# orybkin/video-gcp

Measured on AMD Instinct MI355X. Metric: predicted frames/sec, 64x64x3 seq_len=80 gcp_tree (posterior forward + all loss terms, model(inputs) and model.loss() of train.py:157-159, batch-stat BatchNorm), higher is better.
Workload: dtype f32 (encoder / decoder convs and the tree GEMMs from 512 rows: split-f16 MFMA with f32 accumulate, f32-equivalent; everything else exact f32 MFMA)

## Files before the change

### include/gcpx.h

```cpp
#ifndef GCPX_H
#define GCPX_H

#include <stdint.h>

#ifdef __cplusplus
extern "C" {
#endif

#define GCPX_VERSION 1

typedef enum gcpx_status {
    GCPX_OK = 0,
    GCPX_ERR_INVALID_ARG = -1,
    GCPX_ERR_UNSUPPORTED = -2,
    GCPX_ERR_HIP = -3,
    GCPX_ERR_COMM = -4
} gcpx_status;

typedef enum gcpx_act { GCPX_ACT_NONE = 0, GCPX_ACT_LRELU = 1, GCPX_ACT_TANH = 2 } gcpx_act;

int gcpx_version(void);
const char* gcpx_last_error(void);
int gcpx_conv_grid(void);

typedef struct gcpx_conv_src {
    const float* ptr;
    const float* scale;
    const float* shift;
    int32_t C;
    int32_t frame_div;
    int32_t act;
    int32_t _pad;
} gcpx_conv_src;

typedef enum gcpx_head_mode {
    GCPX_HEAD_RAW = 0,
    GCPX_HEAD_DLM_MEAN = 1,
    GCPX_HEAD_DLM_BOTH = 2,
    GCPX_HEAD_TANH_NCHW = 3,
    GCPX_HEAD_DLM_NLL = 4,
    GCPX_HEAD_DLM_NLL_GRAD = 5
} gcpx_head_mode;

typedef struct gcpx_conv_args {
    gcpx_conv_src src[2];
    int32_t nsrc;
    int32_t F;
    int32_t Hin, Win;
    int32_t Hout, Wout;
    int32_t Cin;
    int32_t Cout;
    int32_t out_pitch;
    int32_t upsample;
    int32_t out_act;
    int32_t head_mode;
    const float* wpk;
    const float* bias;
    float* out;
    float* images;
    float* stats_partial;
    const int32_t* raw_row_map;
    const int32_t* src_row_map;
    const int32_t* src_row_frames;
    int32_t n_src_rows;
    int32_t w_split_log2;
    const void* wpk_split;
    const int32_t* w_split_log2_dev;
    int32_t split_layout;
    int32_t nll_rows;
    const float* nll_target;
    float* nll_partial;
    const float* nll_row_weight;
    float nll_scale;
    int32_t _pad3;
    float* images_rows;
    int64_t images_rows_dup;
    const float* bwd_r;
    const float *bwd_scale, *bwd_shift, *bwd_mean, *bwd_rstd;
    const float* addend;
    int32_t addend_frame_div;
    int32_t _pad4;
} gcpx_conv_args;

typedef enum gcpx_split_layout { GCPX_SPLIT_PLAIN = 0, GCPX_SPLIT_ROWFOLD = 1, GCPX_SPLIT_HEAD32 = 2 } gcpx_split_layout;

int gcpx_conv3x3(const gcpx_conv_args* a, void* stream);
int gcpx_conv3x3_grid(const gcpx_conv_args* a);
int gcpx_conv4x4s2(const gcpx_conv_args* a, void* stream);
int gcpx_conv4x4s2_grid(void);
int gcpx_conv4x4s2_image(const float* x, const float* wpk, const float* bias, float* out,
                         int32_t F, int32_t Hin, int32_t Win, int32_t Cout, int32_t out_act, void* stream);

int gcpx_bn_finalize(const float* partial, int32_t n_partial, int32_t pitch, int32_t C, double count,
                     const float* gamma, const float* beta, float eps, float* scale, float* shift,
                     float* running_mean, float* running_var, float momentum, float* mean_out, float* rstd_out,
                     void* stream);
int gcpx_randn(float* out, int64_t n, uint64_t* state, void* stream);
int gcpx_bn_fold(const float* running_mean, const float* running_var, const float* gamma, const float* beta,
                 float eps, int32_t C, float* scale, float* shift, void* stream);

typedef struct gcpx_row_src {
    const float* ptr;
    const int32_t* rowidx;
    const float* scale;
    const float* shiftv;
    int64_t sb, sr;
    int32_t width;
    int32_t shift;
    int32_t act;
    int32_t cmod;
} gcpx_row_src;

typedef enum gcpx_gemm_epi {
    GCPX_EPI_NONE = 0,
    GCPX_EPI_LRELU = 1,
    GCPX_EPI_LSTM = 2,
    GCPX_EPI_GAUSS_SAMPLE = 3
} gcpx_gemm_epi;

struct gcpx_lstm_bwd_args;
typedef struct gcpx_gemm_args {
    gcpx_row_src src[6];
    int32_t nsrc;
    int32_t M, N, K, rpb;
    const float* wpk;
    const float* bias;
    float* out;
    int64_t ob, orow;
    int32_t epi;
    int32_t nbatch;
    float* stats_partial;
    const float* c_prev;
    int64_t c_prev_stride;
    float* h_out;
    float* c_out;
    int64_t hb, hrow;
    float* h_copy;
    int64_t z_src_off, z_w_off, z_bias_off, z_out_off;
    float* gates_out;
    const void* wpk_split;
    const int32_t* w_split_log2_dev;
    int32_t w_split_log2;
    int32_t _pad_split;
    void* x_planes;
    int32_t* x_exp;
    int64_t x_planes_bytes;
    const struct gcpx_lstm_bwd_args* lstm_bwd;
} gcpx_gemm_args;

int gcpx_gemm(const gcpx_gemm_args* a, void* stream);
int gcpx_gemm_planes_workspace(int32_t M, int32_t K, int32_t nbatch, int64_t* planes_bytes, int64_t* n_exp);
int gcpx_gemm_group_dims(const gcpx_gemm_args* host_table, int32_t n, int32_t* dims, int32_t* total_blocks);
int gcpx_gemm_group(const gcpx_gemm_args* dev_table, const int32_t* dev_dims, int32_t n, int32_t total_blocks, void* stream);
int gcpx_gemm_row_blocks(int32_t M, int32_t N);

typedef enum gcpx_mlp_epi { GCPX_MLP_PLAIN = 0, GCPX_MLP_GAUSS = 1,
                             GCPX_MLP_TANH = 2  } gcpx_mlp_epi;

typedef struct gcpx_mlp_args {
    gcpx_row_src src[6];
    int32_t nsrc;
    int32_t M, rpb;
    int32_t in_dim, mid, n_mid, out_dim;
    const float* w_in;
    const float* b_in;
    const float* w_mid;
    const float* b_mid;
    const float* gn_gamma;
    const float* gn_beta;
    const float* w_out;
    const float* b_out;
    float gn_eps;
    float lrelu_slope;
    int32_t epi;
    int32_t out_split;
    float* out;
    int64_t ob, orow, oblk;
    const float* eps;
    int64_t eb, erow;
    float* z;
    int64_t zb, zrow;
    float* save;
} gcpx_mlp_args;

int gcpx_mlp(const gcpx_mlp_args* a, void* stream);
int gcpx_mlp_group_dims(const gcpx_mlp_args* host_table, int32_t n, int32_t* dims, int32_t* total_blocks);
int gcpx_mlp_group(const gcpx_mlp_args* dev_table, const int32_t* dev_dims, int32_t n, int32_t total_blocks, int32_t mid,
                   void* stream);
int gcpx_mlp_group_gemm_supported(const gcpx_gemm_args* g, int32_t total_blocks, int32_t mid);
int gcpx_mlp_group_gemm(const gcpx_mlp_args* dev_table, const int32_t* dev_dims, int32_t n, int32_t total_blocks, int32_t mid,
                        const gcpx_gemm_args* g, void* stream);

int gcpx_balanced_binding(const int64_t* end_ind, int32_t B, int32_t L, int32_t T, int32_t* node_t,
                          int32_t* leave, int32_t* frame2node, int32_t* etilde_row, int32_t* seq_len,
                          int32_t* node2row, void* stream);

int gcpx_gather_rows(const float* src, const int32_t* idx, float* out, int32_t B, int32_t T, int32_t N,
                     int32_t idx_offset, int64_t row_floats, void* stream);
int gcpx_gather_rows_rest(const float* src, const int32_t* idx, float* out, int32_t B, int32_t T, int32_t N, int32_t idx_offset,
                          int64_t row_floats, const int32_t* written, void* stream);
int gcpx_seq_pairs(const float* lat, const int32_t* lengths, const float* goal, float* nxt, int32_t n, int32_t T,
                   int32_t nz, void* stream);
int gcpx_masked_row_sum(const float* vals, const int32_t* lengths, float* out, int32_t n, int32_t T, void* stream);
int gcpx_rollout_cost(const float* x, int64_t ld, const int32_t* lengths, const float* goal, int64_t goal_stride, float* out, int32_t n,
                      int32_t T, int32_t D, int32_t kind, int32_t dense, float final_step_weight, void* stream);
int gcpx_copy_rows(const float* src, float* dst, int32_t B, int32_t rows, int64_t row_floats, int64_t src_batch_rows,
                   int64_t dst_batch_rows, void* stream);
int gcpx_gauss_sample(const float* muls, int64_t mb, int64_t mr, const float* eps, int64_t eb, int64_t er, float* z,
                      int64_t zb, int64_t zr, int32_t M, int32_t rpb, int32_t nz, void* stream);
int gcpx_seq_index(const int64_t* end_ind, int32_t B, int32_t T, int32_t* idx, int32_t* seq_len, void* stream);
int gcpx_fill_zero(void* ptr, int64_t nbytes, void* stream);
int gcpx_compact_index(const int32_t* leave, int32_t B, int32_t N, int32_t T, int32_t* dst_idx, void* stream);

typedef struct gcpx_loss_args {
    const float* nll_bt;
    const float* pad_mask;
    const float* kl_b;
    const float* len_logits;
    const int64_t* end_ind;
    const float* existence;
    const int32_t* leave;
    const float* regressed_state;
    const float* state_target;
    const int32_t* seq_len;
    float* out;
    int32_t B, T, N, state_dim;
    float w_rec, w_kl, w_len, w_exist, w_state;
    float total_div;
    const float* action_pred;
    const float* action_seq;
    const int64_t* inv_t0;
    const float* cost_pred;
    const float* cost_target;
    int32_t n_actions;
    float w_action, w_cost;
    const float* state_mask;
    const float* w_kl_dev;
} gcpx_loss_args;

int gcpx_dlm_nll(const float* params, const float* target, const float* row_weight, float* nll_out, int32_t rows,
                 int32_t npix, int32_t pitch, int32_t n_mix, void* stream);
int gcpx_gauss_nll(const float* mu, const float* target, const float* log_sigma, float* nll_out, int32_t rows,
                   int32_t nelem, void* stream);
int gcpx_kl_gauss(const float* qz, const float* pz, int32_t B, int32_t N, int32_t nz, int64_t batch_stride,
                  int64_t node_stride, float free_nats, const float* node_weight ,
                  int64_t weight_bstride, float* kl_out, void* stream);
int gcpx_loss_combine(const gcpx_loss_args* a, void* stream);
int gcpx_loss_pre(const gcpx_loss_args* a, const float* qz, const float* pz, int32_t N, int32_t nz, int64_t batch_stride,
                  int64_t node_stride, float free_nats, const float* node_weight, int64_t weight_bstride, float* kl_out, void* stream);
int gcpx_loss_final(const gcpx_loss_args* a, void* stream);


int gcpx_aux_sample_indices(const int64_t* end_ind, const float* u, int32_t B, int32_t temp_dist, int64_t* inv_t0, int64_t* inv_t1,
                            int64_t* cost_start, int64_t* cost_end, void* stream);
int gcpx_aux_sample_indices_gauss(const int64_t* end_ind, const float* n, int32_t B, int32_t temp_dist, int64_t* inv_t0, int64_t* inv_t1,
                                  int64_t* cost_start, int64_t* cost_end, void* stream);
int gcpx_aux_index_rows(const int64_t* inv_t0, const int64_t* inv_t1, const int64_t* cost_start, const int64_t* cost_end, int32_t B,
                        int32_t T, int32_t Wd, int32_t* rows, void* stream);
int gcpx_path_cost(const float* x, const int64_t* start_idx, const int64_t* end_idx, int32_t B, int32_t T, int32_t rows,
                   int32_t row_len, float* partial, float* out, void* stream);
int gcpx_sample_length(const float* logits, const float* u, int32_t B, int32_t T, int32_t min_len, int64_t* end_ind, void* stream);


int gcpx_image_metrics(const float* est, const float* tgt, const int32_t* frame_map, const int32_t* first, const int32_t* last,
                       int32_t B, int32_t T, int32_t C, int32_t H, int32_t W, double* scratch, float* out, void* stream);

int gcpx_topn_accumulate(const float* metrics, int32_t B, int32_t n, int32_t N, int32_t comp, int32_t lower_is_better, float* all,
                         int32_t* best, const float* pool, int32_t pool_rows, const int32_t* frame_map, const int32_t* first,
                         const int32_t* last, int32_t T, float* best_frames, const float* full_pool, int32_t full_rows,
                         const int32_t* full_map, int32_t F, float* best_full, int64_t row_floats, void* stream);



typedef enum gcpx_wgrad_mode {
    GCPX_WG_ROWS = 0,
    GCPX_WG_CONV1D = 1,
    GCPX_WG_CONV3X3 = 2,
    GCPX_WG_CONV4X4S2 = 3
} gcpx_wgrad_mode;
typedef enum gcpx_wgrad_map {
    GCPX_WMAP_LINEAR = 0,
    GCPX_WMAP_CONV = 1,
    GCPX_WMAP_CONVT = 2
} gcpx_wgrad_map;

typedef struct gcpx_wgrad_args {
    const float* dy;
    const float* x;
    const int32_t* rowidx;
    const int32_t* frame_map;
    const float* scale;
    const float* shiftv;
    float* out;
    int64_t ldy, sb, sr, ldw;
    int64_t dy_sb;
    int32_t R, N, n_valid;
    int32_t K, mode, Cin, H, W, rpb, shift, act, cmod;
    int32_t k_off, accumulate, partial, nsplit;
    int32_t dy_rpb;
    int32_t nbatch;
    float* dbias;
// ... 293 lines not shown
```

### video-gcp_amd/csrc/gemm.hip

```cpp
#include "common.h"
#include "gemm_tile.h"

#include <cstdio>
#include <cstdlib>
#include <type_traits>

bool gcpx_gemm_split_applies(const gcpx_gemm_args* a);
int gcpx_launch_gemm_split(const gcpx_gemm_args* a, hipStream_t stream);
bool gcpx_gemm_planes_applies(const gcpx_gemm_args* a);
int gcpx_launch_gemm_planes(const gcpx_gemm_args* a, hipStream_t stream);

namespace {

template <int PR, int CR, bool LSTM, bool KS = false>
__global__ void __launch_bounds__(256) gemm_kernel(const gcpx_gemm_args a) {
    gemm_tile<PR, CR, LSTM, KS>(a, blockIdx.x, blockIdx.y, blockIdx.z);
}

__global__ void __launch_bounds__(256) gemm_group_kernel(const gcpx_gemm_args* __restrict__ tab, const int4* __restrict__ dims, const int n) {
    int p = 0;
    while (p + 1 < n && (int)blockIdx.x >= dims[p + 1].x) ++p;
    const int4 d = dims[p];
    const int local = blockIdx.x - d.x;
    const int bx = local % d.y, by = (local / d.y) % d.z, bz = local / (d.y * d.z);
    const gcpx_gemm_args& a = tab[p];
    if (a.epi == GCPX_EPI_GAUSS_SAMPLE) {
        const int r = bx * 16 + ((int)threadIdx.x >> 4), d = by * 16 + ((int)threadIdx.x & 15);
        if (r < a.M) {
            const int b = r / a.rpb, j = r % a.rpb;
            const float* m = a.src[0].ptr + (size_t)b * a.src[0].sb + (size_t)j * a.src[0].sr;
            const float e = a.src[1].ptr[(size_t)b * a.src[1].sb + (size_t)j * a.src[1].sr + d];
            a.out[(size_t)b * a.ob + (size_t)j * a.orow + d] = m[d] + expf(m[a.N + d]) * e;
        }
        return;
    }
    if (a.epi == GCPX_EPI_LSTM) gemm_tile<1, 1, true, true>(a, bx, by, bz);
    else gemm_tile<1, 1, false, true>(a, bx, by, bz);
}

struct TileChoice { int pr, cr; };

TileChoice choose_tile(int M, int N, int nb = 1) {
    if (const char* ov = getenv("GCPX_GEMM_TILE")) {
        int pr = 0, cr = 0, mm = 0;
        if (sscanf(ov, "%d,%d,%d", &pr, &cr, &mm) == 3 && M >= mm && N % (16 * cr) == 0) return TileChoice{pr, cr};
    }
    static const long simds = [] {
        int dev = 0, cus = 256;
        if (hipGetDevice(&dev) == hipSuccess) (void)hipDeviceGetAttribute(&cus, hipDeviceAttributeMultiprocessorCount, dev);
        return 4L * (cus > 0 ? cus : 256);
    }();
    const int prs[3] = {4, 2, 1}, crs[3] = {4, 2, 1};
    TileChoice best{1, 1};
    double best_cost = -1.0, best_bytes = 0.0;
    const long NT = N / 16, RT = (M + 15) / 16;
    if (M >= 64 && N % 64 == 0 && ((RT + 3) / 4) * (NT / 4) * nb >= simds) return TileChoice{4, 4};
    for (int pi = 0; pi < 3; ++pi)
        for (int ci = 0; ci < 3; ++ci) {
            const int pr = prs[pi], cr = crs[ci];
            if (N % (16 * cr)) continue;
            if (pr > 1 && 16 * pr > ((M + 15) & ~15)) continue;
            const long waves = ((RT + pr - 1) / pr) * ((NT + cr - 1) / cr) * nb;
            const long rounds = (waves + simds - 1) / simds;
            const int area = pr * cr;
            const double e = area >= 16 ? 4.2 : area >= 8 ? 4.9 : area >= 4 ? 5.0 : area >= 2 ? 6.0 : 8.0;
            const double compute = (double)rounds * area * e * (rounds > 1 ? 1.35 : 1.0);
            const double bytes = 256.0 * (pr + cr) / area;
            const double l2 = (double)RT * NT * nb * 256.0 * bytes / 1.0e7;
            const double cost = compute > l2 ? compute : l2;
            if (best_cost < 0 || cost < best_cost - 1e-9 || (cost < best_cost + 1e-9 && bytes < best_bytes)) {
                best_cost = cost; best_bytes = bytes; best = TileChoice{pr, cr};
            }
        }
    return best;
}

template <int PR, int CR>
void launch_t(const gcpx_gemm_args* a, hipStream_t stream) {
    const int rbk = (a->M + 16 * PR - 1) / (16 * PR);
    const int cbk = (a->N / 16 + 4 * CR - 1) / (4 * CR);
    const int nb = a->nbatch > 1 ? a->nbatch : 1;
    if (a->epi == GCPX_EPI_LSTM)
        hipLaunchKernelGGL((gemm_kernel<PR, CR, true>), dim3(rbk, cbk, nb), dim3(256), 0, stream, *a);
    else
        hipLaunchKernelGGL((gemm_kernel<PR, CR, false>), dim3(rbk, cbk, nb), dim3(256), 0, stream, *a);
}

}

extern "C" int gcpx_gemm_row_blocks(int32_t M, int32_t N) {
    const TileChoice t = choose_tile(M, N);
    return (M + 16 * t.pr - 1) / (16 * t.pr);
}

static int gemm_check(const gcpx_gemm_args* a);

static bool ks_block_choice(const gcpx_gemm_args* a, int* pr_out, int* cr_out) {
    static const int max_rows = [] { const char* e = getenv("GCPX_GEMM_KS_MAX_ROWS"); return e ? atoi(e) : 4096; }();
    static const int max_cost = [] { const char* e = getenv("GCPX_GEMM_KS_MAX_COST"); return e ? atoi(e) : 6; }();
    if (!(a->M >= 64 && a->M <= max_rows && a->K >= 256 && !a->stats_partial) || getenv("GCPX_GEMM_NO_KS_BLOCKS")) return false;
    static const long cus = [] {
        int dev = 0, n = 256;
        if (hipGetDevice(&dev) == hipSuccess) (void)hipDeviceGetAttribute(&n, hipDeviceAttributeMultiprocessorCount, dev);
        return (long)(n > 0 ? n : 256);
    }();
    const long nb = a->nbatch > 1 ? a->nbatch : 1;
    const int shapes[5][2] = {{1, 1}, {1, 2}, {2, 2}, {4, 2}, {2, 4}};
    int best = 0;
    long best_cost = -1;
    for (int i = 0; i < 5; ++i) {
        const int pr = shapes[i][0], cr = shapes[i][1];
        if (a->N % (16 * cr)) continue;
        const long wgs = (long)((a->M + 16 * pr - 1) / (16 * pr)) * (a->N / (16 * cr)) * nb;
        const long cost = ((wgs + cus - 1) / cus) * (pr + cr);
        if (best_cost < 0 || cost < best_cost) { best_cost = cost; best = i; }
    }
    if (best == 0 || best_cost > max_cost) return false;
    *pr_out = shapes[best][0];
    *cr_out = shapes[best][1];
    return true;
}

static bool gemm_is_small(const gcpx_gemm_args* a) {
    int pr_ = 1, cr_ = 1;
    if (ks_block_choice(a, &pr_, &cr_)) return false;
    const int nb = a->nbatch > 1 ? a->nbatch : 1;
    const TileChoice t = choose_tile(a->M, a->N, nb);
    const long rbk = (a->M + 15) / 16, nt = a->N / 16;
    return t.pr == 1 && t.cr == 1 && a->K >= 256 && rbk * nt * nb <= 1024 && !a->stats_partial;
}

extern "C" int gcpx_gemm_group_dims(const gcpx_gemm_args* host_table, int32_t n, int32_t* dims, int32_t* total_blocks) {
    GCPX_CHECK_ARG(host_table && dims && total_blocks && n >= 1 && n <= 16, "bad arguments");
    int start = 0;
    for (int p = 0; p < n; ++p) {
        if (host_table[p].epi == GCPX_EPI_GAUSS_SAMPLE) {
            const gcpx_gemm_args& a = host_table[p];
            GCPX_CHECK_ARG(a.nsrc == 2 && a.src[0].ptr && a.src[1].ptr && a.out && a.M > 0 && a.N > 0 && a.N % 16 == 0 && a.rpb > 0 &&
                               a.src[0].width == 2 * a.N && a.src[1].width == a.N, "gauss sample: [mu | log_sigma] rows, eps rows, out");
            dims[4 * p] = start; dims[4 * p + 1] = (a.M + 15) / 16; dims[4 * p + 2] = a.N / 16; dims[4 * p + 3] = 1;
            start += dims[4 * p + 1] * dims[4 * p + 2];
            continue;
        }
        const int st = gemm_check(host_table + p);
        if (st != GCPX_OK) return st;
        if (!gemm_is_small(host_table + p)) {
            gcpx_set_error("gcpx_gemm_group_dims: problem %d (M=%d N=%d K=%d) is not in the small-M split-K regime", p, host_table[p].M,
                           host_table[p].N, host_table[p].K);
            return GCPX_ERR_UNSUPPORTED;
        }
        const int nb = host_table[p].nbatch > 1 ? host_table[p].nbatch : 1;
        const int rbk = (host_table[p].M + 15) / 16, nt = host_table[p].N / 16;
        dims[4 * p] = start; dims[4 * p + 1] = rbk; dims[4 * p + 2] = nt; dims[4 * p + 3] = nb;
        start += rbk * nt * nb;
    }
    *total_blocks = start;
    return GCPX_OK;
}

extern "C" int gcpx_gemm_group(const gcpx_gemm_args* dev_table, const int32_t* dev_dims, int32_t n, int32_t total_blocks, void* stream_) {
    hipStream_t stream = reinterpret_cast<hipStream_t>(stream_);
    GCPX_CHECK_ARG(dev_table && dev_dims && n >= 1 && n <= 16 && total_blocks > 0, "bad arguments");
    GCPX_CHECK_ARG((((uintptr_t)dev_dims) & 15) == 0, "dims must be 16-byte aligned");
    hipLaunchKernelGGL(gemm_group_kernel, dim3(total_blocks), dim3(256), 0, stream, dev_table, reinterpret_cast<const int4*>(dev_dims), n);
    GCPX_CHECK_LAUNCH();
    return GCPX_OK;
}

static int gemm_check(const gcpx_gemm_args* a) {
    GCPX_CHECK_ARG(a != nullptr, "null args");
    GCPX_CHECK_ARG(a->epi != GCPX_EPI_GAUSS_SAMPLE, "GCPX_EPI_GAUSS_SAMPLE is a gcpx_gemm_group problem");
    GCPX_CHECK_ARG(a->nsrc >= 1 && a->nsrc <= 6, "nsrc out of range");
    GCPX_CHECK_ARG(a->M > 0 && a->N > 0 && a->N % 16 == 0 && a->rpb > 0, "bad M/N/rpb");
    int ksum = 0;
    for (int s = 0; s < a->nsrc; ++s) {
        GCPX_CHECK_ARG(a->src[s].ptr != nullptr, "source pointer is NULL");
        GCPX_CHECK_ARG(a->src[s].width > 0 && a->src[s].width % 16 == 0, "source width must be a multiple of 16");
        GCPX_CHECK_ARG(!(a->src[s].scale || a->src[s].act) ||
                           (a->src[s].cmod > 0 && (a->src[s].cmod & (a->src[s].cmod - 1)) == 0),
                       "cmod must be a power of two when scale/act is set");
        ksum += a->src[s].width;
    }
    GCPX_CHECK_ARG(ksum == a->K, "K != sum of source widths");
    GCPX_CHECK_ARG(a->wpk != nullptr, "weights missing");
    if (a->epi == GCPX_EPI_LSTM) {
        GCPX_CHECK_ARG(a->c_prev && a->h_out && a->c_out, "LSTM epilogue needs c_prev/h_out/c_out");
    } else {
        GCPX_CHECK_ARG(a->out != nullptr, "out is NULL");
    }
    GCPX_CHECK_ARG(a->nbatch <= 1 || (a->epi != GCPX_EPI_LSTM && !a->stats_partial), "nbatch > 1 only for plain epilogues");
    GCPX_CHECK_ARG(!a->lstm_bwd || (a->epi == GCPX_EPI_NONE && a->nbatch <= 1 && !a->stats_partial),
                   "lstm_bwd: plain epilogue, single problem");
    return GCPX_OK;
}

bool gcpx_gemm_tile_plan(const gcpx_gemm_args* a, int* pr, int* cr, int* ks, int* gx, int* gy, int* gz) {
    if (gemm_check(a) != GCPX_OK || a->stats_partial) return false;
    const int nb = a->nbatch > 1 ? a->nbatch : 1;
    *gz = nb;
    if (ks_block_choice(a, pr, cr)) {
        *ks = 1; *gx = (a->M + 16 * *pr - 1) / (16 * *pr); *gy = a->N / (16 * *cr);
        return true;
    }
    if (gcpx_gemm_split_applies(a)) return false;
    const TileChoice t = choose_tile(a->M, a->N, nb);
    const long rbk = (a->M + 15) / 16, nt = a->N / 16;
    if (t.pr == 1 && t.cr == 1 && a->K >= 256 && !getenv("GCPX_GEMM_NOKS") && rbk * nt * nb <= 1024) {
        *pr = 1; *cr = 1; *ks = 1; *gx = (int)rbk; *gy = (int)nt;
        return true;
    }
    *pr = t.pr; *cr = t.cr; *ks = 0;
    *gx = (a->M + 16 * t.pr - 1) / (16 * t.pr); *gy = (a->N / 16 + 4 * t.cr - 1) / (4 * t.cr);
    return true;
}

extern "C" int gcpx_gemm(const gcpx_gemm_args* a, void* stream_) {
    hipStream_t stream = reinterpret_cast<hipStream_t>(stream_);
    const int st = gemm_check(a);
    if (st != GCPX_OK) return st;
    {
        int pr_ = 1, cr_ = 1;
        if (!ks_block_choice(a, &pr_, &cr_)) {
            if (gcpx_gemm_planes_applies(a)) return gcpx_launch_gemm_planes(a, stream);
            if (gcpx_gemm_split_applies(a)) return gcpx_launch_gemm_split(a, stream);
        }
    }
    const TileChoice t = choose_tile(a->M, a->N, a->nbatch > 1 ? a->nbatch : 1);
    {
        int pr = 1, cr = 1;
        if (ks_block_choice(a, &pr, &cr)) {
            const long nb = a->nbatch > 1 ? a->nbatch : 1;
            const dim3 grid((a->M + 16 * pr - 1) / (16 * pr), a->N / (16 * cr), nb);
            const bool lstm = a->epi == GCPX_EPI_LSTM;
#define GCPX_KS_LAUNCH(PR_, CR_)                                                                                              \
            do {                                                                                                              \
                if (lstm) hipLaunchKernelGGL((gemm_kernel<PR_, CR_, true, true>), grid, dim3(256), 0, stream, *a);            \
                else hipLaunchKernelGGL((gemm_kernel<PR_, CR_, false, true>), grid, dim3(256), 0, stream, *a);                \
            } while (0)
            if (pr == 1 && cr == 2) GCPX_KS_LAUNCH(1, 2);
            else if (pr == 2 && cr == 2) GCPX_KS_LAUNCH(2, 2);
            else if (pr == 4 && cr == 2) GCPX_KS_LAUNCH(4, 2);
            else GCPX_KS_LAUNCH(2, 4);
#undef GCPX_KS_LAUNCH
            GCPX_CHECK_LAUNCH();
            return GCPX_OK;
        }
    }
    if (t.pr == 1 && t.cr == 1 && a->K >= 256 && !getenv("GCPX_GEMM_NOKS")) {
        const long nb = a->nbatch > 1 ? a->nbatch : 1;
        const long rbk = (a->M + 15) / 16, nt = a->N / 16;
        if (rbk * nt * nb <= 1024) {
            if (a->epi == GCPX_EPI_LSTM)
                hipLaunchKernelGGL((gemm_kernel<1, 1, true, true>), dim3(rbk, nt, nb), dim3(256), 0, stream, *a);
            else
                hipLaunchKernelGGL((gemm_kernel<1, 1, false, true>), dim3(rbk, nt, nb), dim3(256), 0, stream, *a);
            GCPX_CHECK_LAUNCH();
            return GCPX_OK;
        }
    }
    switch (t.pr * 10 + t.cr) {
        case 44: launch_t<4, 4>(a, stream); break;
        case 42: launch_t<4, 2>(a, stream); break;
        case 41: launch_t<4, 1>(a, stream); break;
        case 24: launch_t<2, 4>(a, stream); break;
        case 22: launch_t<2, 2>(a, stream); break;
        case 21: launch_t<2, 1>(a, stream); break;
        case 14: launch_t<1, 4>(a, stream); break;
        case 12: launch_t<1, 2>(a, stream); break;
        default: launch_t<1, 1>(a, stream); break;
    }
    GCPX_CHECK_LAUNCH();
    return GCPX_OK;
}
```

### video-gcp_amd/csrc/gemm_planes.hip

```cpp
#include "common.h"

#include <cstdlib>

#ifndef GP_ABLATE
#define GP_ABLATE 0
#endif

namespace {

typedef _Float16 h8 __attribute__((ext_vector_type(8)));
typedef const f32x4 __attribute__((address_space(1)))* gptr4;
__device__ __forceinline__ float4 gload4(const float* p) {
    const f32x4 t = *(gptr4)p;
    return make_float4(t[0], t[1], t[2], t[3]);
}

__device__ __forceinline__ f32x4 mfma32h(h8 a, h8 b, f32x4 c) {
    return __builtin_amdgcn_mfma_f32_16x16x32_f16(a, b, c, 0, 0, 0);
}

__host__ __device__ __forceinline__ int padded_row_tiles(const int M) { return ((M + 255) >> 8) << 4; }

__device__ __forceinline__ float sigmoid_hw(const float x) { return __builtin_amdgcn_rcpf(1.f + __builtin_amdgcn_exp2f(-1.44269504088896341f * x)); }
__device__ __forceinline__ float tanh_hw(const float x) { return 1.f - 2.f * __builtin_amdgcn_rcpf(1.f + __builtin_amdgcn_exp2f(2.88539008177792681f * x)); }

__device__ __forceinline__ void transpose4_rows(float (&x)[4]) {
    unsigned u[4] = {__float_as_uint(x[0]), __float_as_uint(x[1]), __float_as_uint(x[2]), __float_as_uint(x[3])};
#pragma unroll
    for (int c = 0; c < 2; ++c) {
        auto s = __builtin_amdgcn_permlane32_swap(u[c], u[c + 2], false, false);
        u[c] = s[0]; u[c + 2] = s[1];
    }
#pragma unroll
    for (int c = 0; c < 4; c += 2) {
        auto s = __builtin_amdgcn_permlane16_swap(u[c], u[c + 1], false, false);
        u[c] = s[0]; u[c + 1] = s[1];
    }
#pragma unroll
    for (int c = 0; c < 4; ++c) x[c] = __uint_as_float(u[c]);
}

template <bool XF, int NWV>
__global__ void __launch_bounds__(64 * NWV) split_rows_kernel(const gcpx_gemm_args a) {
    __shared__ unsigned wmax[NWV][16];
    const int tid = threadIdx.x, lane = tid & 63, wave = tid >> 6;
    const int j = lane & 15, q = lane >> 4;
    const int zb = blockIdx.z, rt = blockIdx.x;
    const int M = a.M, rpb = a.rpb;
    const int NKS = a.K >> 5;
    const int r = rt * 16 + j;
    const bool rv = r < M;
    const int rs = rv ? r : 0;
    const int rb = rs / rpb, rj = rs % rpb;

    auto for_each_chunk = [&](auto&& f) __attribute__((always_inline)) {
        int s0 = 0;
#pragma unroll
        for (int i = 0; i < 6; ++i) {
            if (i < a.nsrc) {
                const gcpx_row_src& src = a.src[i];
                bool ok = rv;
                size_t off;
                if (src.rowidx) {
                    off = (size_t)src.rowidx[rs] * src.sr;
                } else {
                    const int jj = rj + src.shift;
                    ok = ok && jj >= 0 && jj < rpb;
                    off = (size_t)rb * src.sb + (size_t)(ok ? jj : 0) * src.sr;
                }
                const float* p = src.ptr + (size_t)zb * a.z_src_off + off + q * 8;
                const float mask = ok ? 1.f : 0.f;
                const int n = src.width >> 5;
                for (int l = (wave - s0) & (NWV - 1); l < n; l += NWV) {
                    float4 v0 = gload4(p + 32 * l), v1 = gload4(p + 32 * l + 4);
                    if constexpr (XF) {
                        if (src.scale || src.act) {
                            const int c = (32 * l + q * 8) & (src.cmod - 1);
                            v0 = affine_act4(v0, src.scale, src.shiftv, c, src.act);
                            v1 = affine_act4(v1, src.scale, src.shiftv, (c + 4) & (src.cmod - 1), src.act);
                        }
                    }
                    v0.x *= mask; v0.y *= mask; v0.z *= mask; v0.w *= mask;
                    v1.x *= mask; v1.y *= mask; v1.z *= mask; v1.w *= mask;
                    f(s0 + l, v0, v1);
                }
                s0 += n;
            }
        }
    };

    float amax = 0.f;
    for_each_chunk([&](const int, const float4 v0, const float4 v1) {
        amax = fmaxf(amax, fmaxf(fmaxf(fmaxf(fabsf(v0.x), fabsf(v0.y)), fmaxf(fabsf(v0.z), fabsf(v0.w))),
                                 fmaxf(fmaxf(fabsf(v1.x), fabsf(v1.y)), fmaxf(fabsf(v1.z), fabsf(v1.w)))));
    });
    {
        unsigned u = __float_as_uint(amax);
        auto s16 = __builtin_amdgcn_permlane16_swap(u, u, false, false);
        u = max(s16[0], s16[1]);
        auto s32 = __builtin_amdgcn_permlane32_swap(u, u, false, false);
        u = max(s32[0], s32[1]);
        if (q == 0) wmax[wave][j] = u;
        __syncthreads();
        u = wmax[0][j];
#pragma unroll
        for (int w = 1; w < NWV; ++w) u = max(u, wmax[w][j]);
        amax = __uint_as_float(u);
    }
    const int ew = a.w_split_log2_dev ? a.w_split_log2_dev[zb] : a.w_split_log2;
    const int ex_cap = min(100, 126 - ew);
    int ex = ex_cap;
    if (amax > 0.f) ex = min(ex_cap, max(-100, 14 + 127 - (int)((__float_as_uint(amax) >> 23) & 0xff)));
    if (!(amax < 3.0e38f)) ex = -100;
    const float sc = __uint_as_float((unsigned)(127 + ex) << 23);
    const int RTP = padded_row_tiles(M);
    char* dst = reinterpret_cast<char*>(a.x_planes) + (((size_t)zb * RTP + rt) * NKS) * 2048 + lane * 16;
    for_each_chunk([&](const int ks, const float4 v0, const float4 v1) {
        const float f[8] = {v0.x * sc, v0.y * sc, v0.z * sc, v0.w * sc, v1.x * sc, v1.y * sc, v1.z * sc, v1.w * sc};
        h8 p1, p2;
#pragma unroll
        for (int e = 0; e < 8; ++e) {
            p1[e] = (_Float16)f[e];
            p2[e] = (_Float16)fmaf((float)p1[e], -1.f, f[e]);
        }
        *reinterpret_cast<h8*>(dst + (size_t)ks * 2048) = p1;
        *reinterpret_cast<h8*>(dst + (size_t)ks * 2048 + 1024) = p2;
    });
    if (wave == 0 && q == 0) a.x_exp[(size_t)zb * RTP * 16 + r] = ex;
}

__device__ __forceinline__ void glds16(const char* base, const unsigned voff, const unsigned lds_dst) {
    unsigned keep;
    asm volatile("s_mov_b32 %0, m0\n\ts_mov_b32 m0, %3\n\ts_nop 0\n\tglobal_load_lds_dwordx4 %1, %2\n\ts_mov_b32 m0, %0"
                 : "=&s"(keep) : "v"(voff), "s"(base), "s"(lds_dst) : "memory");
}
template <int N>
__device__ __forceinline__ void wait_vm() {
    asm volatile("s_waitcnt vmcnt(%0)" ::"n"(N) : "memory");
}

template <int RT, int CTN, int NW, int WR, int KSUB, int STAGES, bool LSTM>
__global__ void __launch_bounds__(64 * NW) gemm_planes_kernel(const gcpx_gemm_args a, const int nbx, const int nby) {
    constexpr int WC = NW / WR, RPW = RT / WR, CPW = CTN / WC;
    constexpr int SUB_PIECES = (RT + CTN) * 2;
    constexpr int SUB_BYTES = SUB_PIECES * 1024, STAGE_BYTES = KSUB * SUB_BYTES;
    constexpr int LW = KSUB * CTN * 2 / NW, LX = KSUB * RT * 2 / NW, LPS = LW + LX;
    static_assert((KSUB * CTN * 2) % NW == 0 && (KSUB * RT * 2) % NW == 0 && (CTN * 2) % LW == 0 && (RT * 2) % LX == 0 && LX % 2 == 0 &&
                  RT % WR == 0 && CTN % WC == 0, "tile");
    extern __shared__ float4 smem4[];
    char* smem = reinterpret_cast<char*>(smem4);
    const int tid = threadIdx.x, lane = tid & 63;
    const int wave = __builtin_amdgcn_readfirstlane(tid >> 6);
    const int wr = wave / WC, wc = wave % WC;
    const int j = lane & 15, q = lane >> 4;
    int id = blockIdx.x;
    {
        const int nblk = nbx * nby, qn = nblk >> 3, rn = nblk & 7, xcd = id & 7, idx = id >> 3;
        id = (xcd < rn ? xcd * (qn + 1) : rn * (qn + 1) + (xcd - rn) * qn) + idx;
    }
    const int by = id % nby, bx = id / nby;
    const int zb = blockIdx.z;
    const int NT = a.N >> 4, NKS = a.K >> 5, NK = NKS / KSUB;
    const int M = a.M, rpb = a.rpb;
    const int RTP = padded_row_tiles(M);
    const unsigned lds0 = (unsigned)(uintptr_t)smem;
    const unsigned voff = lane * 16;
    const int gw = wave * LW, gx = wave * LX;
    const int sub_w = gw / (CTN * 2), rem_w = gw % (CTN * 2), sub_x = gx / (RT * 2), rem_x = gx % (RT * 2);
    const char* wv0 = reinterpret_cast<const char*>(a.wpk_split) + (size_t)zb * a.z_w_off * 4 + ((size_t)sub_w * NT + by * CTN) * 2048 + rem_w * 1024;
    const char* xv0 = reinterpret_cast<const char*>(a.x_planes) +
                      ((((size_t)zb * RTP + (size_t)bx * RT + (rem_x >> 1)) * NKS) + sub_x) * 2048;
    const size_t wstride = (size_t)KSUB * NT * 2048, xrow = (size_t)NKS * 2048;
    const unsigned dw0 = lds0 + sub_w * SUB_BYTES + rem_w * 1024, dx0 = lds0 + sub_x * SUB_BYTES + (CTN * 2 + rem_x) * 1024;

    auto issue = [&](const int s, const int b) __attribute__((always_inline)) {
        const char* wp = wv0 + (size_t)s * wstride;
        const char* xp = xv0 + (size_t)s * (KSUB * 2048);
        const unsigned db = b * STAGE_BYTES;
#pragma unroll
        for (int i = 0; i < LW; ++i) glds16(wp + i * 1024, voff, dw0 + db + i * 1024);
#pragma unroll
        for (int i = 0; i < LX; ++i) glds16(xp + (size_t)(i >> 1) * xrow + (i & 1) * 1024, voff, dx0 + db + i * 1024);
    };

    f32x4 acc[CPW][RPW];
#pragma unroll
    for (int c = 0; c < CPW; ++c)
#pragma unroll
        for (int i = 0; i < RPW; ++i) acc[c][i] = f32x4{0, 0, 0, 0};

    auto compute = [&](const int b) __attribute__((always_inline)) {
        const char* base = smem + b * STAGE_BYTES + lane * 16;
#pragma unroll
        for (int sub = 0; sub < KSUB; ++sub) {
            const char* sb = base + sub * SUB_BYTES;
            const char* xb = sb + CTN * 2048 + (wr * RPW * 2) * 1024;
            h8 w[CPW][2], x[3][2];
#pragma unroll
            for (int i = 0; i < 2 && i < RPW; ++i) {
                x[i][0] = *reinterpret_cast<const h8*>(xb + (i * 2) * 1024);
                x[i][1] = *reinterpret_cast<const h8*>(xb + (i * 2 + 1) * 1024);
            }
#pragma unroll
            for (int c = 0; c < CPW; ++c) {
                const char* wp = sb + ((wc * CPW + c) * 2) * 1024;
                w[c][0] = *reinterpret_cast<const h8*>(wp);
                w[c][1] = *reinterpret_cast<const h8*>(wp + 1024);
            }
            __builtin_amdgcn_sched_group_barrier(0x100, 2 * CPW + (RPW < 2 ? 2 : 4), 0);
#pragma unroll
            for (int i = 0; i < RPW; ++i) {
                if (i + 2 < RPW) {
                    x[(i + 2) % 3][0] = *reinterpret_cast<const h8*>(xb + ((i + 2) * 2) * 1024);
                    x[(i + 2) % 3][1] = *reinterpret_cast<const h8*>(xb + ((i + 2) * 2 + 1) * 1024);
                    __builtin_amdgcn_sched_group_barrier(0x100, 2, 0);
                }
#pragma unroll
                for (int c = 0; c < CPW; ++c) acc[c][i] = mfma32h(w[c][1], x[i % 3][0], acc[c][i]);
#pragma unroll
                for (int c = 0; c < CPW; ++c) acc[c][i] = mfma32h(w[c][0], x[i % 3][1], acc[c][i]);
#pragma unroll
                for (int c = 0; c < CPW; ++c) acc[c][i] = mfma32h(w[c][0], x[i % 3][0], acc[c][i]);
                __builtin_amdgcn_sched_group_barrier(0x008, 3 * CPW, 0);
            }
        }
    };

#pragma unroll
    for (int s = 0; s < STAGES - 1; ++s)
        if (s < NK) issue(s, s);
    int buf = 0;
    for (int s = 0; s < NK; ++s) {
        if (s + STAGES - 2 < NK) wait_vm<(STAGES - 2) * LPS>();
        else wait_vm<0>();
        __builtin_amdgcn_s_barrier();
#if GP_ABLATE != 1
        if (s + STAGES - 1 < NK) issue(s + STAGES - 1, buf == 0 ? STAGES - 1 : buf - 1);
#endif
        __builtin_amdgcn_sched_barrier(0);
#ifdef GP_TRACE
        const long long tr0 = __builtin_amdgcn_s_memtime();
        __builtin_amdgcn_sched_barrier(0);
#endif
#if GP_ABLATE != 2
        compute(buf);
#endif
        __builtin_amdgcn_sched_barrier(0);
#ifdef GP_TRACE
        if (blockIdx.x == 0 && zb == 0 && lane == 0) {
            long long* tr = reinterpret_cast<long long*>(a.h_copy) + ((size_t)wave * NK + s) * 2;
            tr[0] = tr0;
            tr[1] = __builtin_amdgcn_s_memtime();
        }
        __builtin_amdgcn_sched_barrier(0);
#endif
        buf = buf + 1 == STAGES ? 0 : buf + 1;
    }

    const int ew = a.w_split_log2_dev ? a.w_split_log2_dev[zb] : a.w_split_log2;
    const int nt0 = by * CTN + wc * CPW;
    if constexpr (LSTM && CPW == 4) {
        const bool al = ((reinterpret_cast<uintptr_t>(a.c_prev) | reinterpret_cast<uintptr_t>(a.h_out) | reinterpret_cast<uintptr_t>(a.c_out) |
                          reinterpret_cast<uintptr_t>(a.h_copy)) & 15) == 0 && ((a.c_prev_stride | a.hb | a.hrow) & 3) == 0;
        if (al) {
            float4 bv[CPW];
#pragma unroll
            for (int c = 0; c < CPW; ++c) {
                bv[c] = make_float4(0.f, 0.f, 0.f, 0.f);
                if (a.bias) bv[c] = *reinterpret_cast<const float4*>(a.bias + (size_t)zb * a.z_bias_off + (nt0 + c) * 16 + q * 4);
            }
            const int u4 = (nt0 + q) * 4;
#pragma unroll
            for (int i = 0; i < RPW; ++i) {
                const int r = (bx * RT + wr * RPW + i) * 16 + j;
                const bool rv = r < M;
                const int rs = rv ? r : 0;
                const int rb = rs / rpb, rj = rs % rpb;
                const int ex = a.x_exp[(size_t)zb * RTP * 16 + rs];
                const float inv = __uint_as_float((unsigned)(127 - ex - ew) << 23);
                const float4 cp4 = *reinterpret_cast<const float4*>(a.c_prev + (size_t)rs * a.c_prev_stride + u4);
                float cp[4] = {cp4.x, cp4.y, cp4.z, cp4.w}, hv[4], cv[4];
                transpose4_rows(cp);
#pragma unroll
                for (int c = 0; c < CPW; ++c) {
                    const f32x4 v = acc[c][i];
                    const float ig = sigmoid_hw(fmaf(v[0], inv, bv[c].x)), fg = sigmoid_hw(fmaf(v[1], inv, bv[c].y));
                    const float gg = tanh_hw(fmaf(v[2], inv, bv[c].z)), og = sigmoid_hw(fmaf(v[3], inv, bv[c].w));
                    cv[c] = fg * cp[c] + ig * gg;
                    hv[c] = og * tanh_hw(cv[c]);
                    if (a.gates_out && rv)
                        *reinterpret_cast<float4*>(a.gates_out + ((size_t)r * (a.N / 4) + (nt0 + c) * 4 + q) * 4) = make_float4(ig, fg, gg, og);
                }
                transpose4_rows(hv);
                transpose4_rows(cv);
                if (rv) {
                    const size_t o = (size_t)rb * a.hb + (size_t)rj * a.hrow + u4;
                    *reinterpret_cast<float4*>(a.h_out + o) = make_float4(hv[0], hv[1], hv[2], hv[3]);
                    *reinterpret_cast<float4*>(a.c_out + o) = make_float4(cv[0], cv[1], cv[2], cv[3]);
#ifndef GP_TRACE
                    if (a.h_copy) *reinterpret_cast<float4*>(a.h_copy + (size_t)r * (a.N / 4) + u4) = make_float4(hv[0], hv[1], hv[2], hv[3]);
#endif
                }
            }
            return;
        }
    }
#pragma unroll
    for (int i = 0; i < RPW; ++i) {
        const int r = (bx * RT + wr * RPW + i) * 16 + j;
        const bool rv = r < M;
        const int rs = rv ? r : 0;
        const int rb = rs / rpb, rj = rs % rpb;
        const int ex = a.x_exp[(size_t)zb * RTP * 16 + rs];
        const float inv = __uint_as_float((unsigned)(127 - ex - ew) << 23);
#pragma unroll
        for (int c = 0; c < CPW; ++c) {
            const int nt = nt0 + c;
            const int n = nt * 16 + q * 4;
            float4 bv = make_float4(0.f, 0.f, 0.f, 0.f);
            if (a.bias) bv = *reinterpret_cast<const float4*>(a.bias + (size_t)zb * a.z_bias_off + n);
            f32x4 v = acc[c][i];
            v[0] = fmaf(v[0], inv, bv.x); v[1] = fmaf(v[1], inv, bv.y); v[2] = fmaf(v[2], inv, bv.z); v[3] = fmaf(v[3], inv, bv.w);
            if (!rv) continue;
            if constexpr (LSTM) {
                const int u = nt * 4 + q;
                const float cp = a.c_prev[(size_t)r * a.c_prev_stride + u];
                const float ig = sigmoid_hw(v[0]), fg = sigmoid_hw(v[1]), gg = tanh_hw(v[2]), og = sigmoid_hw(v[3]);
                const float cn = fg * cp + ig * gg;
                const float h = og * tanh_hw(cn);
                const size_t o = (size_t)rb * a.hb + (size_t)rj * a.hrow + u;
                a.h_out[o] = h;
                a.c_out[o] = cn;
                if (a.gates_out) *reinterpret_cast<float4*>(a.gates_out + ((size_t)r * (a.N / 4) + u) * 4) = make_float4(ig, fg, gg, og);
#ifndef GP_TRACE
                if (a.h_copy) a.h_copy[(size_t)r * (a.N / 4) + u] = h;
#endif
            } else {
                if (a.epi == GCPX_EPI_LRELU) {
                    v[0] = lrelu(v[0], 0.2f); v[1] = lrelu(v[1], 0.2f); v[2] = lrelu(v[2], 0.2f); v[3] = lrelu(v[3], 0.2f);
                }
                float* op = a.out + (size_t)zb * a.z_out_off + (size_t)rb * a.ob + (size_t)rj * a.orow + n;
                *reinterpret_cast<float4*>(op) = make_float4(v[0], v[1], v[2], v[3]);
            }
        }
    }
}

template <int RT, int CTN, int NW, int WR, int KSUB, int STAGES>
int launch_planes(const gcpx_gemm_args* a, hipStream_t stream) {
    constexpr int LDS = STAGES * KSUB * (RT + CTN) * 2048;
    static bool attr_set = false;
    if (!attr_set) {
        for (const void* k : {reinterpret_cast<const void*>(gemm_planes_kernel<RT, CTN, NW, WR, KSUB, STAGES, false>),
                              reinterpret_cast<const void*>(gemm_planes_kernel<RT, CTN, NW, WR, KSUB, STAGES, true>)}) {
            hipError_t e = hipFuncSetAttribute(k, hipFuncAttributeMaxDynamicSharedMemorySize, LDS);
            if (e != hipSuccess) {
                gcpx_set_error("gemm planes: hipFuncSetAttribute(%d B LDS): %s", LDS, hipGetErrorString(e));
                return GCPX_ERR_HIP;
            }
        }
        attr_set = true;
    }
    const int nb = a->nbatch > 1 ? a->nbatch : 1;
    const int nbx = (a->M + RT * 16 - 1) / (RT * 16), nby = a->N / (CTN * 16);
    const dim3 grid(nbx * nby, 1, nb);
    if (a->epi == GCPX_EPI_LSTM)
        hipLaunchKernelGGL((gemm_planes_kernel<RT, CTN, NW, WR, KSUB, STAGES, true>), grid, dim3(64 * NW), LDS, stream, *a, nbx, nby);
    else
        hipLaunchKernelGGL((gemm_planes_kernel<RT, CTN, NW, WR, KSUB, STAGES, false>), grid, dim3(64 * NW), LDS, stream, *a, nbx, nby);
    GCPX_CHECK_LAUNCH();
    return GCPX_OK;
}

}

extern "C" int gcpx_gemm_planes_workspace(int32_t M, int32_t K, int32_t nbatch, int64_t* planes_bytes, int64_t* n_exp) {
    const int64_t nb = nbatch > 1 ? nbatch : 1;
    const int64_t rtp = padded_row_tiles(M);
    if (planes_bytes) *planes_bytes = nb * rtp * (K / 32) * 2048;
    if (n_exp) *n_exp = nb * rtp * 16;
    return GCPX_OK;
}

bool gcpx_gemm_planes_applies(const gcpx_gemm_args* a) {
    static const int min_rows = [] { const char* e = getenv("GCPX_GEMM_PLANES_MIN_ROWS"); return e ? atoi(e) : 512; }();
    if (!a->x_planes || !a->x_exp || !a->wpk_split || a->M < min_rows || a->N % 128 || a->K % 64 || a->stats_partial || a->lstm_bwd) return false;
    for (int s = 0; s < a->nsrc; ++s)
        if (a->src[s].width % 32) return false;
    int64_t need = 0;
    gcpx_gemm_planes_workspace(a->M, a->K, a->nbatch, &need, nullptr);
    return a->x_planes_bytes >= need;
}

int gcpx_launch_gemm_planes(const gcpx_gemm_args* a, hipStream_t stream) {
    const int nb = a->nbatch > 1 ? a->nbatch : 1;
    bool xf = false;
    for (int s = 0; s < a->nsrc; ++s) xf = xf || a->src[s].scale || a->src[s].act;
    const dim3 sgrid((a->M + 15) / 16, 1, nb);
    if ((long)sgrid.x * nb >= 1024) {
        if (xf) hipLaunchKernelGGL((split_rows_kernel<true, 4>), sgrid, dim3(256), 0, stream, *a);
        else hipLaunchKernelGGL((split_rows_kernel<false, 4>), sgrid, dim3(256), 0, stream, *a);
    } else {
        if (xf) hipLaunchKernelGGL((split_rows_kernel<true, 16>), sgrid, dim3(1024), 0, stream, *a);
        else hipLaunchKernelGGL((split_rows_kernel<false, 16>), sgrid, dim3(1024), 0, stream, *a);
    }
    GCPX_CHECK_LAUNCH();
    static const int force = [] { const char* e = getenv("GCPX_GEMM_PLANES_CFG"); return e ? atoi(e) : 0; }();
    const long tiles_a = (long)((a->M + 255) / 256) * (a->N / 256) * nb, tiles_b = (long)((a->M + 127) / 128) * (a->N / 256) * nb;
    const long tiles_d = (long)((a->M + 127) / 128) * (a->N / 128) * nb;
    const bool n256 = a->N % 256 == 0;
    if (force == 1 && n256) return launch_planes<16, 16, 8, 2, 1, 2>(a, stream);
    if (force == 2 && n256) return launch_planes<8, 16, 8, 2, 1, 3>(a, stream);
    if (force == 3) return launch_planes<8, 8, 8, 4, 2, 2>(a, stream);
    if (force == 4) return launch_planes<4, 8, 4, 2, 2, 3>(a, stream);
    if (force == 5) return launch_planes<16, 8, 8, 4, 1, 3>(a, stream);
    if (force == 6) return launch_planes<8, 8, 8, 4, 1, 4>(a, stream);
    if (force == 7) return launch_planes<4, 4, 4, 4, 2, 4>(a, stream);
    if (n256 && tiles_a >= 256) return launch_planes<16, 16, 8, 2, 1, 2>(a, stream);
    if (n256 && tiles_b >= 256) return launch_planes<8, 16, 8, 2, 1, 3>(a, stream);
    if (tiles_d >= 256) return launch_planes<8, 8, 8, 4, 2, 2>(a, stream);
    const long tiles_c = (long)((a->M + 63) / 64) * (a->N / 128) * nb;
    if (tiles_c < 192) return launch_planes<4, 4, 4, 4, 2, 4>(a, stream);
    return launch_planes<4, 8, 4, 2, 2, 3>(a, stream);
}
```

### video-gcp_amd/csrc/mlp.hip

```cpp
#include "common.h"
#include "gemm_tile.h"

#include <cstdlib>

bool gcpx_gemm_tile_plan(const gcpx_gemm_args* a, int* pr, int* cr, int* ks, int* gx, int* gy, int* gz);

namespace {

template <int MID, bool LEAN>
__device__ __forceinline__ void mlp_rows(const gcpx_mlp_args& a, const int bx, const int by, const int ny, float* hid) {
    constexpr int NTM = MID / 16;
    constexpr int NW = NTM >= 4 ? 4 : NTM;
    constexpr int TPW = NTM / NW;
    constexpr int PITCH = MID + 4;
    constexpr int CPG = MID / 8;
    static_assert(CPG == 4 || CPG == 16, "GroupNorm group must be one lane (4) or one 16-channel tile");

    const int lane = threadIdx.x & 63, wave = threadIdx.x >> 6;
    const int j = lane & 15, q = lane >> 4;
    const int r = bx * 16 + j;
    const bool rv = r < a.M;
    const int rs = rv ? r : 0;
    const int rb = rs / a.rpb, rj = rs % a.rpb;
    const float slope = a.lrelu_slope;
// ... 207 lines not shown
            }
            if (rv) {
                const int n = nt * 16 + q * 4;
                if (n < a.out_dim) {
                    const float4 bv = *reinterpret_cast<const float4*>(a.b_out + n);
                    float v[4] = {ao[0] + bv.x, ao[1] + bv.y, ao[2] + bv.z, ao[3] + bv.w};
                    if (a.epi == GCPX_MLP_TANH) { v[0] = tanhf(v[0]); v[1] = tanhf(v[1]); v[2] = tanhf(v[2]); v[3] = tanhf(v[3]); }
                    const int blk = n / split, nn = n % split;
                    float* op = orow + (size_t)blk * a.oblk + nn;
                    if (n + 3 < a.out_dim && nn + 3 < split && (((uintptr_t)op) & 15) == 0) {
                        *reinterpret_cast<float4*>(op) = make_float4(v[0], v[1], v[2], v[3]);
                    } else {
#pragma unroll
                        for (int k = 0; k < 4; ++k) {
                            const int nk = n + k;
                            if (nk < a.out_dim) orow[(size_t)(nk / split) * a.oblk + nk % split] = v[k];
                        }
                    }
                }
            }
        }
    }
}

__device__ __forceinline__ void prefetch_range(const float* base, const size_t n_floats, const int slot, const int nslots) {
    const size_t n4 = n_floats / 4;
    const float4* p = reinterpret_cast<const float4*>(base);
    for (size_t i = (size_t)slot * 256 + threadIdx.x; i < n4; i += (size_t)nslots * 256) {
        const float4 v = p[i];
        asm volatile("" ::"v"(v.x), "v"(v.y), "v"(v.z), "v"(v.w));
    }
}

__device__ __forceinline__ void prefetch_weights(const gcpx_mlp_args& a, const int helper, const int nhelpers) {
    const int nslots = nhelpers >= 8 ? nhelpers / 8 : 1;
    const int slot = nhelpers >= 8 ? helper / 8 : helper;
    if (slot >= nslots) return;
    const int out_pad = (a.out_dim + 15) & ~15;
    prefetch_range(a.w_in, (size_t)a.in_dim * a.mid, slot, nslots);
    if (a.n_mid) prefetch_range(a.w_mid, (size_t)a.n_mid * a.mid * a.mid, slot, nslots);
    prefetch_range(a.w_out, (size_t)a.mid * out_pad, slot, nslots);
}

template <int MID, bool LEAN>
__global__ void __launch_bounds__(256, LEAN ? 2 : 1) mlp_kernel(const gcpx_mlp_args a, const int nblocks) {
    __shared__ float4 hid4[2 * 16 * (MID + 4) / 4];
    const int gx = (a.M + 15) / 16;
    if ((int)blockIdx.x >= nblocks) {
        prefetch_weights(a, blockIdx.x - nblocks, gridDim.x - nblocks);
        return;
    }
    mlp_rows<MID, LEAN>(a, blockIdx.x % gx, blockIdx.x / gx, nblocks / gx, reinterpret_cast<float*>(hid4));
}

template <int MID, bool LEAN>
__global__ void __launch_bounds__(256, LEAN ? 2 : 1) mlp_group_kernel(const gcpx_mlp_args* __restrict__ tab, const int4* __restrict__ dims, const int n,
                                                                      const int nblocks) {
    __shared__ float4 hid4[2 * 16 * (MID + 4) / 4];
    if ((int)blockIdx.x >= nblocks) {
        for (int p = 0; p < n; ++p) prefetch_weights(tab[p], blockIdx.x - nblocks, gridDim.x - nblocks);
        return;
    }
    int p = 0;
    while (p + 1 < n && (int)blockIdx.x >= dims[p + 1].x) ++p;
    const int4 d = dims[p];
    const int local = blockIdx.x - d.x;
    mlp_rows<MID, LEAN>(tab[p], local % d.y, local / d.y, d.z, reinterpret_cast<float*>(hid4));
}

template <int MID, int PR, int CR, bool KS>
__global__ void __launch_bounds__(256, 1) level_pre_kernel(const gcpx_mlp_args* __restrict__ tab, const int4* __restrict__ dims, const int n,
                                                           const int nblocks, const gcpx_gemm_args g, const int gx, const int gy, const int gz) {
    __shared__ float4 hid4[2 * 16 * (MID + 4) / 4];
    const int blk = blockIdx.x;
    if (blk >= nblocks) {
        const int local = blk - nblocks, ng = gx * gy * gz;
        if (local < ng) {
            gemm_tile<PR, CR, false, KS>(g, local % gx, (local / gx) % gy, local / (gx * gy));
        } else {
            for (int p = 0; p < n; ++p) prefetch_weights(tab[p], local - ng, gridDim.x - nblocks - ng);
        }
        return;
    }
    int p = 0;
    while (p + 1 < n && blk >= dims[p + 1].x) ++p;
    const int4 d = dims[p];
    const int local = blk - d.x;
    mlp_rows<MID, false>(tab[p], local % d.y, local / d.y, d.z, reinterpret_cast<float*>(hid4));
}

typedef void (*level_pre_fn)(const gcpx_mlp_args*, const int4*, int, int, const gcpx_gemm_args, int, int, int);
level_pre_fn level_pre_variant(const int pr, const int cr, const int ks) {
    if (ks) {
        if (pr == 1 && cr == 1) return level_pre_kernel<128, 1, 1, true>;
        if (pr == 1 && cr == 2) return level_pre_kernel<128, 1, 2, true>;
        if (pr == 2 && cr == 2) return level_pre_kernel<128, 2, 2, true>;
        if (pr == 4 && cr == 2) return level_pre_kernel<128, 4, 2, true>;
        if (pr == 2 && cr == 4) return level_pre_kernel<128, 2, 4, true>;
        return nullptr;
    }
    if (pr == 2 && cr == 2) return level_pre_kernel<128, 2, 2, false>;
    if (pr == 4 && cr == 2) return level_pre_kernel<128, 4, 2, false>;
    return nullptr;
}

int mlp_check(const gcpx_mlp_args* a) {
    GCPX_CHECK_ARG(a != nullptr, "null args");
    GCPX_CHECK_ARG(a->nsrc >= 1 && a->nsrc <= 6, "nsrc out of range");
    GCPX_CHECK_ARG(a->M > 0 && a->rpb > 0, "bad M/rpb");
    int ksum = 0;
    for (int s = 0; s < a->nsrc; ++s) {
        GCPX_CHECK_ARG(a->src[s].ptr != nullptr, "source pointer is NULL");
        GCPX_CHECK_ARG(a->src[s].width > 0 && a->src[s].width % 16 == 0, "source width must be a multiple of 16");
        ksum += a->src[s].width;
    }
    GCPX_CHECK_ARG(ksum == a->in_dim, "in_dim != sum of source widths");
    GCPX_CHECK_ARG(a->w_in && a->b_in && a->w_out && a->b_out, "weights missing");
    GCPX_CHECK_ARG(a->n_mid == 0 || (a->w_mid && a->b_mid && a->gn_gamma && a->gn_beta), "hidden-layer weights missing");
    if (a->epi == GCPX_MLP_GAUSS) {
        GCPX_CHECK_ARG(a->out_dim % 32 == 0 && a->eps && a->z, "GAUSS epilogue needs out_dim % 32 == 0, eps, z");
    } else {
        GCPX_CHECK_ARG(a->out != nullptr, "out is NULL");
    }
    return GCPX_OK;
}

void mlp_grid(const gcpx_mlp_args* a, int* gx, int* gy) {
    *gx = (a->M + 15) / 16;
    const int head_tiles = ((a->epi == GCPX_MLP_GAUSS ? a->out_dim / 2 : a->out_dim) + 15) / 16;
    static const int ymax = [] { const char* e = getenv("GCPX_MLP_GY_MAX"); return e ? atoi(e) : 32; }();
    int y = 1;
    while (y < ymax && *gx * y < 256 && head_tiles / (4 * y) >= 2) y *= 2;
    *gy = y;
}

int mlp_helpers(const int nb, const int cus) {
    static const int cap = [] { const char* e = getenv("GCPX_MLP_HELPERS"); return e ? atoi(e) : 1 << 30; }();
    if (nb > cus / 4) return 0;
    const int h = ((cus - nb) / 8) * 8;
    return h < cap ? (h > 0 ? h : 0) : cap;
}

}

extern "C" int gcpx_mlp_group_dims(const gcpx_mlp_args* host_table, int32_t n, int32_t* dims, int32_t* total_blocks) {
    GCPX_CHECK_ARG(host_table && dims && total_blocks && n >= 1 && n <= 16, "bad arguments");
    int start = 0;
    for (int p = 0; p < n; ++p) {
        const int st = mlp_check(host_table + p);
        if (st != GCPX_OK) return st;
        GCPX_CHECK_ARG(host_table[p].mid == host_table[0].mid, "all problems of a group share the hidden width");
        int gx, gy;
        mlp_grid(host_table + p, &gx, &gy);
        dims[4 * p] = start; dims[4 * p + 1] = gx; dims[4 * p + 2] = gy; dims[4 * p + 3] = 0;
        start += gx * gy;
    }
    *total_blocks = start;
    return GCPX_OK;
}

extern "C" int gcpx_mlp_group(const gcpx_mlp_args* dev_table, const int32_t* dev_dims, int32_t n, int32_t total_blocks, int32_t mid,
                              void* stream_) {
    hipStream_t stream = reinterpret_cast<hipStream_t>(stream_);
    GCPX_CHECK_ARG(dev_table && dev_dims && n >= 1 && n <= 16 && total_blocks > 0, "bad arguments");
    GCPX_CHECK_ARG((((uintptr_t)dev_dims) & 15) == 0, "dims must be 16-byte aligned");
    const int cus = gcpx_conv_grid() / 2;
    const bool lean = total_blocks > cus;
    const int grid = total_blocks + mlp_helpers(total_blocks, cus);
    const int4* dd = reinterpret_cast<const int4*>(dev_dims);
    if (mid == 128 && lean) hipLaunchKernelGGL((mlp_group_kernel<128, true>), dim3(grid), dim3(256), 0, stream, dev_table, dd, n, total_blocks);
    else if (mid == 128) hipLaunchKernelGGL((mlp_group_kernel<128, false>), dim3(grid), dim3(256), 0, stream, dev_table, dd, n, total_blocks);
    else if (mid == 32 && lean) hipLaunchKernelGGL((mlp_group_kernel<32, true>), dim3(grid), dim3(256), 0, stream, dev_table, dd, n, total_blocks);
    else if (mid == 32) hipLaunchKernelGGL((mlp_group_kernel<32, false>), dim3(grid), dim3(256), 0, stream, dev_table, dd, n, total_blocks);
    else {
        gcpx_set_error("gcpx_mlp_group: unsupported mid=%d (128 or 32)", mid);
        return GCPX_ERR_UNSUPPORTED;
    }
    GCPX_CHECK_LAUNCH();
    return GCPX_OK;
}

extern "C" int gcpx_mlp_group_gemm_supported(const gcpx_gemm_args* g, int32_t total_blocks, int32_t mid) {
    if (!g || mid != 128 || g->epi == GCPX_EPI_LSTM || g->epi == GCPX_EPI_GAUSS_SAMPLE) return 0;
    const int cus = gcpx_conv_grid() / 2;
    if (total_blocks > cus) return 0;
    int pr, cr, ks, gx, gy, gz;
    if (!gcpx_gemm_tile_plan(g, &pr, &cr, &ks, &gx, &gy, &gz)) return 0;
    return level_pre_variant(pr, cr, ks) != nullptr;
}

extern "C" int gcpx_mlp_group_gemm(const gcpx_mlp_args* dev_table, const int32_t* dev_dims, int32_t n, int32_t total_blocks, int32_t mid,
                                   const gcpx_gemm_args* g, void* stream_) {
    hipStream_t stream = reinterpret_cast<hipStream_t>(stream_);
    GCPX_CHECK_ARG(dev_table && dev_dims && g && n >= 1 && n <= 16 && total_blocks > 0, "bad arguments");
    GCPX_CHECK_ARG((((uintptr_t)dev_dims) & 15) == 0, "dims must be 16-byte aligned");
    int pr, cr, ks, gx, gy, gz;
    level_pre_fn kern = nullptr;
    if (mid == 128 && g->epi != GCPX_EPI_LSTM && g->epi != GCPX_EPI_GAUSS_SAMPLE && gcpx_gemm_tile_plan(g, &pr, &cr, &ks, &gx, &gy, &gz))
        kern = level_pre_variant(pr, cr, ks);
    if (!kern) {
        gcpx_set_error("gcpx_mlp_group_gemm: this GEMM / hidden width has no combined launch (ask gcpx_mlp_group_gemm_supported)");
        return GCPX_ERR_UNSUPPORTED;
    }
    const int cus = gcpx_conv_grid() / 2;
    const int work = total_blocks + gx * gy * gz;
    const int grid = work + mlp_helpers(work, cus);
    hipLaunchKernelGGL(kern, dim3(grid), dim3(256), 0, stream, dev_table, reinterpret_cast<const int4*>(dev_dims), n, total_blocks, *g, gx, gy, gz);
    GCPX_CHECK_LAUNCH();
    return GCPX_OK;
}

extern "C" int gcpx_mlp(const gcpx_mlp_args* a, void* stream_) {
    hipStream_t stream = reinterpret_cast<hipStream_t>(stream_);
    const int st = mlp_check(a);
    if (st != GCPX_OK) return st;
    int gx, gy;
    mlp_grid(a, &gx, &gy);
    const int cus = gcpx_conv_grid() / 2;
    const bool lean = gx * gy > cus;
    const int nb = gx * gy, grid = nb + mlp_helpers(nb, cus);
    if (a->mid == 128 && lean) hipLaunchKernelGGL((mlp_kernel<128, true>), dim3(grid), dim3(256), 0, stream, *a, nb);
    else if (a->mid == 128) hipLaunchKernelGGL((mlp_kernel<128, false>), dim3(grid), dim3(256), 0, stream, *a, nb);
    else if (a->mid == 32 && lean) hipLaunchKernelGGL((mlp_kernel<32, true>), dim3(grid), dim3(256), 0, stream, *a, nb);
    else if (a->mid == 32) hipLaunchKernelGGL((mlp_kernel<32, false>), dim3(grid), dim3(256), 0, stream, *a, nb);
    else {
        gcpx_set_error("gcpx_mlp: unsupported mid=%d (128 or 32)", a->mid);
        return GCPX_ERR_UNSUPPORTED;
    }
    GCPX_CHECK_LAUNCH();
    return GCPX_OK;
}
```

### video-gcp_amd/forward_plan.py

```python
import ctypes as C
import os
from contextlib import contextmanager

import torch

from . import packing as pk
from . import runtime as rt
from .hparams import GCPHParams
from .params import init_params, encoder_layers, encoder_skip_layers, decoder_layers
from .plan_ops import _Plan, _addr, N_LANES


class ForwardPlanMixin:

    def _plan_encoder(self, plan, tag, x_ptr, F, out_ptr, out_ob, out_orow, out_rpb):
        hp, P, lib = self._hp, self.pk, self.lib
        G = lib.gcpx_conv4x4s2_grid()
        S = hp.img_sz
        skip_idx = encoder_skip_layers(hp)
        skips = {}
        a0 = self._buf(f"{tag}.a0", (F, S // 2, S // 2, hp.ngf))
        enc_rec = dict(F=F, x_ptr=x_ptr, a0=a0, r={}, out=(out_ptr, out_ob, out_orow, out_rpb))
        plan.rec[f"enc:{tag}"] = enc_rec
        plan.add(f"enc.input:{tag}", lib.gcpx_conv4x4s2_image, x_ptr, P["enc.input.w"].data_ptr(),
# ... 169 lines not shown
                    dMD = self._buf("bw.dMD", (B * T, S_, S_, self._head_pitch))
                    plan.add("zero_unmapped", lib.gcpx_zero_unmapped_rows, dMD.data_ptr(), S_ * S_ * self._head_pitch, r2f.data_ptr(), B * T)

        enc_traj = inf_enc = None
        plan.fork([1, 2])
        traj_first = os.environ.get("GCPX_ENC_ORDER") != "small_first"
        def plan_traj_encoder():
            nonlocal enc_traj, inf_enc
            plan.lane = 0
            if has_traj:
                enc_traj = self._buf("enc_traj", (B * T, nz))
                self._plan_encoder(plan, "traj", tin["traj_seq"].data_ptr(), B * T, enc_traj.data_ptr(), T * nz, nz, T)
                if hp.seq_enc == "none":
                    inf_enc = enc_traj
                else:
                    inf_enc = self._buf("inf_enc_seq", (B * T, nz))
                    self._plan_seq_encoder(plan, "seq", "inf_encoder", enc_traj, inf_enc, B)
                if attentive:
                    dk = hp.nz_attn_key
                    n_mod = L if hp.untied_layers else 1
                    if hp.seq_enc == "none":
                        kenc = enc_traj
                    else:
                        kenc = self._buf("inf_key_enc", (B * T, nz))
                        self._plan_seq_encoder(plan, "kseq", "inf_key_encoder.0", enc_traj, kenc, B)
                    keys = self._buf("inf_enc_key_seq", (B * T, dk))
                    dense = lambda t, w: self._rowsrc(t.data_ptr(), 0, w, w)
                    self._gemm(plan, "kseq.key", [dense(kenc, nz)], B * T, dk, B * T, P["kseq.key.w"], P["kseq.key.b"],
                               out=keys.data_ptr(), ob=0, orow=dk)
                    Kp = self._buf("attn.K", (n_mod, B * T, dk))
                    Vp = self._buf("attn.V", (n_mod, B * T, nz))
                    self._gemm(plan, "attn.k_proj", [dense(keys, dk)], B * T, dk, B * T, P["attn.k_proj.w"], P["attn.k_proj.b"],
                               out=Kp.data_ptr(), ob=0, orow=dk, batch=(n_mod, 0, P["attn.k_proj.w"][0].numel(), dk, B * T * dk))
                    self._gemm(plan, "attn.v_proj", [dense(inf_enc, nz)], B * T, nz, B * T, P["attn.v_proj.w"], P["attn.v_proj.b"],
                               out=Vp.data_ptr(), ob=0, orow=nz, batch=(n_mod, 0, P["attn.v_proj.w"][0].numel(), nz, B * T * nz))
                    plan.rec["attn_kv"] = dict(Kp=Kp, Vp=Vp, keys=keys, kenc=kenc, n_mod=n_mod)

        if traj_first:
            plan_traj_encoder()
        plan.lane = 1
        if "rng_all" in tin:
            plan.add("randn", lib.gcpx_randn, tin["rng_all"].data_ptr(), tin["rng_all"].numel(), self._buf("rng_state", (2,), torch.int64).data_ptr())
            if "aux_n" in tin and not pred_len:
                plan.wait(2, 1)
        skips = self._plan_encoder(plan, "I0", tin["I_0"].data_ptr(), B, _addr(E), PS * nz, 0, 1)
        plan.lane = 2
        if not pred_len:
            if "aux_n" in tin:
                plan_aux_indices()
            plan_bookkeeping()
        if hp.attach_cost_mdl and hp.run_cost_mdl and train_aux and self._has_aux_training:
            gt = self._buf("cost_target", (B,))
            rows = hp.input_nc * hp.img_sz
            plan.add("path_cost", lib.gcpx_path_cost, tin["traj_seq"].data_ptr(), tin["cost_start_idx"].data_ptr(),
                     tin["cost_end_idx"].data_ptr(), B, T, rows, hp.img_sz, self._buf("cost_partial", (B, rows)).data_ptr(), gt.data_ptr())
        self._plan_encoder(plan, "Ig", tin["I_g"].data_ptr(), B, _addr(E, 2 ** L * nz), PS * nz, 0, 1)
        outs = {}
        e0 = lambda: self._rowsrc(_addr(E), PS * nz, 0, nz)
        eg = lambda: self._rowsrc(_addr(E, 2 ** L * nz), PS * nz, 0, nz)
        if hp.regress_length and not pred_len:
            plan.wait(2, 1)
            logits = self._buf("seq_len_logits", (B, T))
            self._mlp(plan, "length_pred", P["length_pred"], [e0(), eg()], B, 1, out=logits.data_ptr(), ob=T, orow=0)
            outs["seq_len_logits"] = logits
        if not traj_first:
            plan_traj_encoder()
        plan.lane = 0
        plan.join([1, 2])

        if hp.regress_length and pred_len:
            logits = self._buf("seq_len_logits", (B, T))
            self._mlp(plan, "length_pred", P["length_pred"], [e0(), eg()], B, 1, out=logits.data_ptr(), ob=T, orow=0)
            outs["seq_len_logits"] = logits
            plan.add("sample_length", lib.gcpx_sample_length, logits.data_ptr(), tin["len_u"].data_ptr(), B, T, 2, tin["end_ind"].data_ptr())
            plan_bookkeeping()

        side_merge = False
        for l in range(L):
            W = P[f"tree{l if hp.untied_layers else 0}"]
            s = 2 ** (L - 1 - l)
            n = 2 ** l
            M = B * n
            nodeoff = lambda w: s * w
            el = lambda: self._rowsrc(_addr(E), PS * nz, 2 * s * nz, nz)
            er = lambda: self._rowsrc(_addr(E, 2 * s * nz), PS * nz, 2 * s * nz, nz)
            pz_out = (_addr(PZ, nodeoff(2 * nv)), PS * 2 * nv, 2 * s * 2 * nv)
            z_map = (_addr(Z, nodeoff(nv)), PS * nv, 2 * s * nv)
            nl = hp.n_lstm_layers
            merged = self._buf(f"merged{l}", (M, 2 * nl * H))

            def plan_merge(lv=l, group=None):
                s_, n_ = 2 ** (L - 1 - lv), 2 ** lv
                Wl = P[f"tree{lv if hp.untied_layers else 0}"]
                mg = self._buf(f"merged{lv}", (B * n_, 2 * nl * H))
                if hp.tree_lstm == "sum":
                    for side, mode in ((0, 0), (2 * s_ * SD, 1)):
                        plan.add(f"merge{lv}.{mode}", lib.gcpx_rows_strided, _addr(mg), n_ * SD, SD, _addr(Hid, side), PS * SD, 2 * s_ * SD,
                                 B, n_, SD, mode)
                    return
                if hp.tree_lstm == "linear":
                    h1 = self._rowsrc(_addr(Hid), PS * SD, 2 * s_ * SD, SD)
                    h2 = self._rowsrc(_addr(Hid, 2 * s_ * SD), PS * SD, 2 * s_ * SD, SD)
                    self._gemm(plan, f"merge{lv}", [h1, h2], B * n_, SD, n_, Wl["proj.w"], Wl["proj.b"], out=_addr(mg), ob=n_ * SD, orow=SD,
                               group=group)
                    return
                h1 = self._rowsrc(_addr(Hid), PS * SD, 2 * s_ * SD, H)
                h2 = self._rowsrc(_addr(Hid, 2 * s_ * SD), PS * SD, 2 * s_ * SD, H)
                self._gemm(plan, f"merge{lv}", [h1, h2], B * n_, H, n_, Wl["proj.w"], Wl["proj.b"], out=_addr(mg),
                           ob=n_ * 2 * nl * H, orow=2 * nl * H, batch=(2 * nl, H, Wl["proj.w"][0].numel(), H, H), group=group)

            merge_with_predictors = not has_z and not sample_prior and hp.tree_lstm not in ("sum", "")
            if has_z:
                g = (_addr(tin["z"], (s - 1) * nv), N * nv, 2 * s * nv) + z_map
                self._mlp(plan, f"prior{l}", W["prior"], [el(), er()], M, n, out=pz_out[0], ob=pz_out[1], orow=pz_out[2], gauss=g)
            elif sample_prior:
                g = (_addr(tin["eps"], (n - 1) * nv), N * nv, nv) + z_map
                self._mlp(plan, f"prior{l}", W["prior"], [el(), er()], M, n, out=pz_out[0], ob=pz_out[1], orow=pz_out[2], gauss=g)
            else:
                pq = []
                self._mlp(plan, f"prior{l}", W["prior"], [el(), er()], M, n, out=pz_out[0], ob=pz_out[1], orow=pz_out[2], group=pq)
                if attentive:
                    et = self._plan_attention(plan, l, W, el(), er(), M, n, B, plan.rec["attn_kv"]["Kp"], plan.rec["attn_kv"]["Vp"], tin)
                else:
                    et = self._rowsrc(inf_enc.data_ptr(), 0, nz, nz, rowidx=etrow[B * (n - 1):])
                g = (_addr(tin["eps"], (n - 1) * nv), N * nv, nv) + z_map
                self._mlp(plan, f"posterior{l}", W["q"], [el(), er(), et], M, n, out=_addr(QZ, nodeoff(2 * nv)),
                          ob=PS * 2 * nv, orow=2 * s * 2 * nv, gauss=g, group=pq)
                mg = []
                if l > 0 and merge_with_predictors and not side_merge:
                    plan_merge(l, group=mg)
                self._mlp_group(plan, f"prior+posterior{l}", pq, gemm=(mg[0] if mg else None))
                if side_merge:
                    plan.join([1])
                    side_merge = False
            zs = lambda: self._rowsrc(z_map[0], z_map[1], z_map[2], nv)
            if not hp.tree_lstm:
                srcs = [el(), er(), zs()] + ([e0(), eg()] if hp.context_every_step else [])
                self._mlp(plan, f"subgoal{l}", W["sg"], srcs, M, n, out=_addr(E, nodeoff(nz)), ob=PS * nz, orow=2 * s * nz, tanh=True)
                continue
            if l == 0:
                if hp.lstm_init == "zero":
                    for slot in (0, 2 ** L):
                        plan.add(f"lstm_init.zero{slot}", lib.gcpx_rows_strided, _addr(Hid, slot * SD), PS * SD, 0, self._zero_row(SD).data_ptr(),
                                 0, 0, B, 1, SD, 0)
                else:
                    self._mlp(plan, "lstm_init", W["init"], [el(), er(), zs()], M, n, out=_addr(Hid), ob=PS * SD, orow=0,
                              oblk=2 ** L * SD, out_split=SD)
                plan_merge()
            x = self._buf(f"x{l}.0", (M, H))
            srcs = [el(), er(), zs()] + ([e0(), eg()] if hp.context_every_step else [])
            fused = "lstm0f.w" in W and not self.save_for_backward
            if not fused:
                self._gemm(plan, f"embed{l}", srcs, M, H, n, W["embed.w"], W["embed.b"], out=x.data_ptr(), ob=n * H, orow=H)
            for i in range(nl):
                xn = self._buf(f"x{l}.{i + 1}", (M, H))
                xs = self._rowsrc(x.data_ptr(), n * H, H, H)
                hs = self._rowsrc(_addr(merged, 2 * i * H), n * 2 * nl * H, 2 * nl * H, H)
                lstm = (_addr(merged, (2 * i + 1) * H), 2 * nl * H, _addr(Hid, nodeoff(SD) + 2 * i * H),
                        _addr(Hid, nodeoff(SD) + (2 * i + 1) * H), PS * SD, 2 * s * SD, xn.data_ptr())
                if i == 0 and fused:
                    self._gemm(plan, f"lstm{l}.0", srcs + [hs], M, 4 * H, n, W["lstm0f.w"], W["lstm0f.b"], epi=rt.EPI_LSTM, lstm=lstm)
                else:
                    self._gemm(plan, f"lstm{l}.{i}", [xs, hs], M, 4 * H, n, W[f"lstm{i}.w"], W[f"lstm{i}.b"],
                               epi=rt.EPI_LSTM, lstm=lstm)
                x = xn
            g = []
            self._gemm(plan, f"out{l}", [self._rowsrc(x.data_ptr(), n * H, H, H)], M, nz, n, W["out.w"], W["out.b"],
                       out=_addr(E, nodeoff(nz)), ob=PS * nz, orow=2 * s * nz, group=g)
            if l + 1 < L and not merge_with_predictors:
                plan_merge(l + 1, group=g)
            self._gemm_group(plan, f"out{l}+merge{l + 1}" if len(g) > 1 else f"out{l}", g)
            if (l + 1 < L and merge_with_predictors and hp.tree_lstm == "split_linear" and B * 2 ** (l + 1) >= self._merge_side_rows):
                plan.fork([1])
                plan.lane = 1
                plan_merge(l + 1)
                plan.lane = 0
                side_merge = True

        F = B * N
        matching = adaptive and has_traj and phase == "train"

        heads = []

        def plan_aux(idx, Wd):
            mes = self._buf("model_enc_seq", (B, Wd, nz))
            plan.add("gather.model_enc_seq", lib.gcpx_gather_rows, E.data_ptr(), idx.data_ptr(), mes.data_ptr(), B, Wd, PS, 1, nz)
            outs["model_enc_seq_padded"] = mes
            if hp.run_state_regressor:
                rs = self._buf("regressed_state", (B, Wd, hp.state_dim))
                self._mlp(plan, "state_regressor", P["state_regressor"], [self._rowsrc(mes.data_ptr(), Wd * nz, nz, nz)],
                          B * Wd, Wd, out=rs.data_ptr(), ob=Wd * hp.state_dim, orow=hp.state_dim, group=heads)
                outs["regressed_state_padded"] = rs
            if hp.attach_inv_mdl and phase == "train" and (sample_prior or hp.train_inv_mdl_full_seq or not has_traj):
                act = self._buf("actions", (B, Wd - 1, hp.n_actions))
                first = enc_traj if has_traj else mes
                s0 = self._rowsrc(first.data_ptr(), (T if has_traj else Wd) * nz, nz, nz)
                s1 = self._rowsrc(_addr(mes, nz), Wd * nz, nz, nz)
                self._mlp(plan, "inv_mdl", P["inv_mdl"], [s0, s1], B * (Wd - 1), Wd - 1, out=act.data_ptr(),
                          ob=(Wd - 1) * hp.n_actions, orow=hp.n_actions, group=heads)
                outs["actions_padded"] = act
            aux_rows = None
            if train_aux and ((hp.attach_inv_mdl and not hp.train_inv_mdl_full_seq) or (hp.attach_cost_mdl and hp.run_cost_mdl)):
                aux_rows = self._buf("aux_rows", (4, B), torch.int32)
                plan.add("aux_index_rows", lib.gcpx_aux_index_rows, tin["inv_t0"].data_ptr(), tin["inv_t1"].data_ptr(),
                         tin["cost_start_idx"].data_ptr(), tin["cost_end_idx"].data_ptr(), B, T, Wd, aux_rows.data_ptr())
                gather = lambda t, i: self._rowsrc(t.data_ptr(), 0, nz, nz, rowidx=aux_rows[i])
            if hp.attach_inv_mdl and train_aux and not hp.train_inv_mdl_full_seq:
                act = self._buf("actions_sampled", (B, hp.n_actions))
                self._mlp(plan, "inv_mdl", P["inv_mdl"], [gather(enc_traj, 0), gather(mes, 1)], B, B, out=act.data_ptr(), ob=0,
                          orow=hp.n_actions, group=heads)
                outs["actions_sampled"] = act
            if hp.attach_cost_mdl and hp.run_cost_mdl and train_aux:
                cost = self._buf("cost_pred", (B, 1))
                self._mlp(plan, "cost_mdl", P["cost_mdl"], [gather(mes, 2), gather(mes, 3)], B, B, out=cost.data_ptr(), ob=0, orow=1,
                          group=heads)
                outs["cost_pred"], outs["cost_target"] = cost, self._buf("cost_target", (B,))

        heads_lane = 0
        if heads_lane:
            plan.fork([1])
        plan.lane = heads_lane
        if adaptive:
            dist = self._buf("distances", (B, N - 1))
            self._mlp(plan, "distance", P["distance"], [self._rowsrc(_addr(E, nz), PS * nz, nz, nz),
                                                        self._rowsrc(_addr(E, 2 * nz), PS * nz, nz, nz)],
                      B * (N - 1), N - 1, out=dist.data_ptr(), ob=N - 1, orow=1)
            pruned_len = self._buf("pruned_len", (B,), torch.int32)
            plan.add("distance_prune", lib.gcpx_distance_prune, dist.data_ptr(), C.c_float(hp.learned_pruning_threshold), None, B, N,
                     leave.data_ptr(), kept_idx.data_ptr(), pruned_len.data_ptr(), None)
            outs["distances"], outs["pruned_len"] = dist, pruned_len
            if not matching:
                plan_aux(kept_idx, N)
                outs["aux_len"] = pruned_len
        else:
            plan_aux(kept_idx, T)
            exist = self._buf("existence", (B, N))
            self._mlp(plan, "existence", P["existence"], [self._rowsrc(_addr(E, nz), PS * nz, nz, nz)], F, N,
                      out=exist.data_ptr(), ob=N, orow=1, group=heads)
            outs["existence"] = exist
        if heads:
            self._mlp_group(plan, "heads", heads)
            heads.clear()
        plan.lane = 0

        def kl_args(kl_b, batch=()):
            return (_addr(QZ, 2 * nv), _addr(PZ, 2 * nv)) + batch + (N, nv, PS * 2 * nv, 2 * nv, C.c_float(hp.free_nats), None, 0, kl_b.data_ptr())

        def loss_args():
            kl_b = self._buf("kl_b", (B,))
            la = rt.LossArgs()
            la.nll_bt, la.pad_mask, la.kl_b = self._buf("nll_bt", (B, T)).data_ptr(), tin["pad_mask"].data_ptr(), kl_b.data_ptr()
            la.len_logits = outs["seq_len_logits"].data_ptr() if "seq_len_logits" in outs else None
            la.end_ind = tin["end_ind"].data_ptr()
            if adaptive:
                la.existence, la.leave = outs["distances"].data_ptr(), outs["distance_target"].data_ptr()
            else:
                la.existence, la.leave = outs["existence"].data_ptr(), leave.data_ptr()
            if "regressed_state_padded" in outs and "traj_seq_states" in tin:
                la.regressed_state, la.state_target = outs["regressed_state_padded"].data_ptr(), tin["traj_seq_states"].data_ptr()
            la.seq_len = seq_len.data_ptr()
            if "actions_sampled" in outs and "actions" in tin:
                la.action_pred, la.action_seq, la.inv_t0 = outs["actions_sampled"].data_ptr(), tin["actions"].data_ptr(), tin["inv_t0"].data_ptr()
                la.n_actions, la.w_action = hp.n_actions, hp.action_rec_weight
            if "cost_pred" in outs:
                la.cost_pred, la.cost_target, la.w_cost = outs["cost_pred"].data_ptr(), outs["cost_target"].data_ptr(), 1.0
            loss_out = self._buf("losses", (16,), zero=True)
            la.out, la.B, la.T, la.N, la.state_dim = loss_out.data_ptr(), B, T, (N - 1 if adaptive else N), hp.state_dim
            la.w_rec, la.w_kl, la.w_len, la.w_exist, la.w_state = hp.dense_img_rec_weight, hp.kl_weight, hp.length_pred_weight, 1.0, 1.0
            if self._kl_w is not None:
                la.w_kl_dev = self._kl_w.data_ptr()
            la.total_div = float(T * hp.input_nc * hp.img_sz * hp.img_sz)
            plan.keep.append(la)
            return la, kl_b

        decode, with_loss = key[8], key[7]
        loss_pre = None
        if with_loss and not adaptive:
            loss_pre = loss_args()
            plan.add("loss.pre", lib.gcpx_loss_pre, C.byref(loss_pre[0]), *kl_args(loss_pre[1]))
        if decode:
            F = B * N
            S = hp.img_sz
            prev = self._plan_decoder_features(plan, self._rowsrc(_addr(E, nz), PS * nz, nz, nz), F, N, skips)
            images = self._buf("images_df", (B, N, hp.input_nc, S, S))
            distr = matched_distr = None
            with_loss = key[7]
            dlm = hp.decoder_distribution == "discrete_logistic_mixture"
            head_out, row_map = None, None
            fused_nll = None
            if dlm:
                mode = rt.HEAD_DLM_MEAN
                if self.materialize_distr or (adaptive and self.save_for_backward and with_loss):
                    mode, distr = rt.HEAD_DLM_BOTH, self._buf("distr_df", (B, N, S, S, self._head_pitch))
                    head_out = distr
                elif self._head_grad_fused(key):
                    mode, row_map = rt.HEAD_DLM_NLL_GRAD, node2row
                    head_out = self._buf("bw.dMD", (B * T, S, S, self._head_pitch))
                    fused_nll = self._buf("nll_partial", ((S // 4) * (S // 16), B * T), zero=True)
                    plan.rec["nll_bwd_fused"] = plan.rec["head_grad_fused"] = True
                elif with_loss and not adaptive and not self.save_for_backward and self._head_nll_fusable():
                    mode, row_map = rt.HEAD_DLM_NLL, node2row
                    fused_nll = self._buf("nll_partial", ((S // 4) * (S // 16), B * T), zero=True)
                elif with_loss and not adaptive:
                    mode, matched_distr = rt.HEAD_DLM_BOTH, self._buf("matched_distr", (B, T, S, S, self._head_pitch))
                    head_out, row_map = matched_distr, node2row
            else:
                mode = rt.HEAD_TANH_NCHW
            a = self._conv_args([prev], F, S, S, S, S, hp.head_channels, self._head_pitch, P["dec.head.w"], P["dec.head.b"],
                                head_out, upsample=0, head_mode=mode, images=images)
            rows_direct = self._rows_direct(key) and (row_map is not None or mode == rt.HEAD_DLM_MEAN)
            rows_images = None
            if rows_direct:
                row_map = node2row
                want_matched = has_traj and phase == "train"
                rows_images = self._buf("rows_images", (2 if want_matched else 1, B, T, hp.input_nc, S, S))
                a.images_rows = rows_images.data_ptr()
                a.images_rows_dup = rows_images[0].numel() if want_matched else 0
# ... 112 lines not shown
```

### video-gcp_amd/model.py

```python
import ctypes as C
import os
from contextlib import contextmanager

import torch

from . import packing as pk
from . import runtime as rt
from .hparams import GCPHParams
from .params import init_params, encoder_layers, encoder_skip_layers, decoder_layers
from .plan_ops import _Plan, Outputs, ModelOutputs, PlanOpsMixin, _addr, N_LANES
from .weights import WeightsMixin
from .forward_plan import ForwardPlanMixin
from .replay import ReplayMixin


class GCPTreeModel(WeightsMixin, PlanOpsMixin, ForwardPlanMixin, ReplayMixin):

    _has_aux_training = True
    _has_pred_length = True
    _rng_in_plan = True

    _n_models = 0
    _stream_pool = {}

    def __init__(self, hp: GCPHParams, params=None, device="cuda", seed=0, materialize_distr=False):
        self._hp = hp
        self.device = torch.device(device)
        self.lib = rt.load_library()
        self._check_hp(hp)
        self._flatten_params(params or self._default_params(hp, seed))
        self.training = True
        self._decode = True
        self._sample_prior = False
        self._use_pred_length = False
        self.materialize_distr = materialize_distr
        self._bufs = {}
        self._plans = {}
        self.pk_split = {}
        self._split_tab = None
        self._gsplit, self._gsplit_tabs = {}, {}
        self._gsplit_live = False
        self._merge_side_rows = 1 << 60
        self._planes_min_rows = 1 << 60
        self._arena = None
        self._plan_listeners = []
        self._rng_seed = None
        self._rng_stream_id = GCPTreeModel._n_models
        GCPTreeModel._n_models += 1
        self.n_steps = 0
        self._kl_w = None
        self.use_graph = {"graph": True, "eager": False}.get(os.environ.get("GCPX_FORWARD_REPLAY", "auto"), "auto")
        pool_key = (self.device.index, os.environ.get("GCPX_MAIN_PRIORITY", "0"))
        pool = None if os.environ.get("GCPX_PRIVATE_STREAMS") else GCPTreeModel._stream_pool.get(pool_key)
        if pool is None:
            main = torch.cuda.Stream(device=self.device, priority=int(os.environ.get("GCPX_MAIN_PRIORITY", "0")))
            lanes = [main.cuda_stream]
            for _ in range(N_LANES - 1):
                sp = C.c_void_p()
                with torch.cuda.device(self.device):
                    rt.check(self.lib.gcpx_stream_create(C.byref(sp)), "stream_create")
                lanes.append(sp)
            pool = (main, lanes)
            if not os.environ.get("GCPX_PRIVATE_STREAMS"):
                GCPTreeModel._stream_pool[pool_key] = pool
        self._stream, self._streams = pool[0], list(pool[1])
        self._set_kl_weight()
        self.save_for_backward = False
        self.split_f16 = os.environ.get("GCPX_EXACT_F32") is None
        self.fused_head_nll = os.environ.get("GCPX_UNFUSED_NLL") is None
        self.head32 = os.environ.get("GCPX_HEAD32", "0") == "1"
        self._timed_op = None
        self._timed_events = []
        self._pack_all()
        from . import handles as Hd
        self.encoder, self.decoder, self.dense_rec = Hd.EncoderHandle(self), Hd.DecoderHandle(self), Hd.DenseRecHandle(self)
        self.tree_module = Hd.TreeModuleHandle(self)
        if hp.attach_inv_mdl:
            self.inv_mdl = Hd.InverseModelHandle(self)
        if hp.attach_cost_mdl:
            self.cost_mdl = Hd.CostModelHandle(self)

    def _check_hp(self, hp):
        assert hp.matching_type in ("balanced", "dtw_image")
        if hp.tree_lstm not in ("split_linear", "linear", "sum", ""):
            raise ValueError("don't know this TreeLSTM type")
        if hp.seq_enc not in ("conv", "none"):
            raise ValueError(f"seq_enc = {hp.seq_enc!r}: 'conv' (ConvSeqEncodingModule) and 'none' (Identity) are built")
        if hp.lstm_init not in ("mlp", "zero"):
            raise ValueError("dont know lstm init type {}!".format(hp.lstm_init))
        if hp.attentive_inference:
            assert hp.n_attention_layers == 1, "one attention layer is built (hyperparameters.py:25 default)"
        assert not (hp.action_conditioned_pred or hp.deterministic or hp.non_goal_conditioned), \
            "the vmpc.py variants belong to the flat predictor (SequentialModel): GCPSequentialModel"
        if hp.adaptive:
            assert hp.top_bias == 1.0 and hp.leaves_bias == 0.0, "WeightsHacker biases are not built (defaults only)"
            assert hp.entropy_weight == 0.0, "the matching entropy is reported, not optimised (hyperparameters.py default)"

    def _n_latents(self):
        return self._hp.n_nodes

    def _zero_row(self, n):
        return self._buf("zero_row", (n,), zero=True)

    def _head_nll_fusable(self):
        hp = self._hp
        return (self.fused_head_nll and self.split_f16 and "dec.head" in self.pk_split and hp.img_sz % 16 == 0 and
                hp.decoder_distribution == "discrete_logistic_mixture" and not self.materialize_distr)

    def _rows_direct(self, key):
        hp = self._hp
        return bool(key[8] and not hp.adaptive and self.split_f16 and "dec.head" in self.pk_split and hp.img_sz % 16 == 0 and
                    hp.decoder_distribution == "discrete_logistic_mixture" and not self.materialize_distr and
                    os.environ.get("GCPX_HEAD_NO_ROWS") is None and type(self)._build_plan is GCPTreeModel._build_plan)

    def _head_grad_fused(self, key):
        has_traj, sample_prior, phase, with_loss = key[1], key[3], key[4], key[7]
        return bool(self.save_for_backward and with_loss and has_traj and not sample_prior and phase == "train" and
                    not self._hp.adaptive and self._head_nll_fusable() and type(self)._build_plan is GCPTreeModel._build_plan)

    def _default_params(self, hp, seed):
        return init_params(hp, seed)

    def train(self, mode=True):
        self.training = mode
        return self

    def eval(self):
        return self.train(False)

    @contextmanager
    def val_mode(self, pred_length=True, decode=True):
        self._sample_prior, self._use_pred_length, self._decode = True, pred_length, decode
        try:
            yield
        finally:
            self._sample_prior, self._use_pred_length, self._decode = False, False, True

    def state_dict(self):
        return dict(self.sd)

    def step(self):
        self.n_steps = self.n_steps + 1
        self._set_kl_weight()

    def _set_kl_weight(self):
        hp = self._hp
        if hp.kl_weight_burn_in:
            w = hp.kl_weight * min(1.0, self.n_steps / float(hp.kl_weight_burn_in))
            if self._kl_w is None:
                self._kl_w = torch.zeros(1, device=self.device)
            self._kl_w.fill_(w)
            self.kl_weight_now = w
        else:
            self._kl_w, self.kl_weight_now = None, hp.kl_weight

    def load_state_dict(self, sd, strict=True):
        for k, v in sd.items():
            if k in self.sd:
                self.sd[k].copy_(v)
            elif strict:
                raise KeyError(k)
        self._pack_all()
        self._clear_plans()

    def _clear_plans(self):
        self._plans.clear()
        for cb in self._plan_listeners:
            cb()

    def __call__(self, inputs, phase="train", noise=None):
        return self.forward(inputs, phase, noise)

    def input_buffer(self, name, shape, dtype=None):
        if dtype is None:
            dtype = torch.int64 if name in ("end_ind", "inv_t0", "inv_t1", "cost_start_idx", "cost_end_idx") else torch.float32
        return self._buf("in." + name, tuple(shape), dtype)

    _buf_prefix = ""

    def _wrap_outputs(self, o, tin, phase):
        hp = self._hp
        out = ModelOutputs()
        out["_model"] = self
        out.end_ind = tin["end_ind"]
        out.raw = o
        out.images_df = o.get("images_df")
        if "seq_len_logits" in o:
            out.seq_len_logits = o["seq_len_logits"]
        if "existence" in o:
            out.existence_predictor = Outputs(existence=o["existence"])
        if "distances" in o:
            out.distance_predictor = Outputs(distances=o["distances"])
        if "soft_matched_estimates" in o:
            out.soft_matched_estimates = o["soft_matched_estimates"]
        if "match_dist_df" in o:
            out.entropy = o["entropy_df"].index_select(1, TreeView.bf2df_index(hp.hierarchy_levels, self.device))
# ... 226 lines not shown
```

### video-gcp_amd/plan_ops.py

```python
import ctypes as C
import os
from contextlib import contextmanager

import torch

from . import packing as pk
from . import runtime as rt
from .hparams import GCPHParams
from .params import init_params, encoder_layers, encoder_skip_layers, decoder_layers


def _addr(t, off_elems=0):
    return t.data_ptr() + 4 * off_elems


N_LANES = 3


class _Plan:

    def __init__(self, lib):
        self.lib = lib
        self.ops = []
        self.keep = []
# ... 20 lines not shown
    def fork(self, lanes):
        self.ops.append(("@fork", None, (tuple(lanes), self._events(1)), 0))

    def join(self, lanes):
        self.ops.append(("@join", None, (tuple(lanes), self._events(len(lanes))), 0))

    def wait(self, waiter, signaler):
        self.ops.append(("@wait", None, (waiter, signaler, self._events(1)[0]), 0))

    def record(self, lane):
        ev = self._events(1)[0]
        self.ops.append(("@record", None, (lane, ev), 0))
        return ev

    def await_event(self, lane, ev):
        self.ops.append(("@await", None, (lane, ev), 0))

    def mark(self, tag, payload):
        self.ops.append(("@mark", None, (tag, payload), 0))

    def compact(self, streams, min_len=3, ranges=None):
        lib, out, run = self.lib, [], []
        inside = (lambda i: True) if ranges is None else (lambda i: any(a <= i < b for a, b in ranges))

        def flush():
            if len(run) >= min_len:
                st = streams[run[0][3]]
                rt.check(lib.gcpx_graph_begin(st), "graph_begin")
                for name, fn, args, _ in run:
                    rt.check(fn(*args, st), name)
                g = C.c_void_p()
                rt.check(lib.gcpx_graph_end(st, C.byref(g)), "graph_end")
                out.append(("@graph", None, (g, tuple(o[0] for o in run)), run[0][3]))
            else:
                out.extend(run)
            run.clear()
        for i, op in enumerate(self.ops):
            ctl = op[0].startswith("@") or not inside(i)
            if ctl or (run and op[3] != run[0][3]):
                flush()
            (out if ctl else run).append(op)
        flush()
        return out

    def run(self, streams, ops=None, on_mark=None):
        lib = self.lib
        for name, fn, args, lane in (self.ops if ops is None else ops):
            if name == "@mark":
                if on_mark is not None:
                    on_mark(*args)
            elif name == "@fork":
                lanes, evs = args
                rt.check(lib.gcpx_event_record(evs[0], streams[0]), "fork")
                for l in lanes:
                    rt.check(lib.gcpx_stream_wait_event(streams[l], evs[0]), "fork")
            elif name == "@wait":
                waiter, signaler, ev = args
                rt.check(lib.gcpx_event_record(ev, streams[signaler]), "wait")
                rt.check(lib.gcpx_stream_wait_event(streams[waiter], ev), "wait")
            elif name == "@graph":
                rt.check(lib.gcpx_graph_launch(args[0], streams[lane]), "graph_launch")
            elif name == "@record":
                rt.check(lib.gcpx_event_record(args[1], streams[args[0]]), "record")
            elif name == "@await":
                rt.check(lib.gcpx_stream_wait_event(streams[args[0]], args[1]), "await")
            elif name == "@join":
                lanes, evs = args
                for l, e in zip(lanes, evs):
                    rt.check(lib.gcpx_event_record(e, streams[l]), "join")
                    rt.check(lib.gcpx_stream_wait_event(streams[0], e), "join")
            else:
                st = fn(*args, streams[lane])
                if st != 0:
                    rt.check(st, name)


class Outputs(dict):
    __getattr__ = dict.__getitem__
    __setattr__ = dict.__setitem__


class ModelOutputs(Outputs):

    _LAZY = ("pruned_prediction", "actions", "regressed_state", "model_enc_seq", "cost", "cost_target")

    def __getattr__(self, name):
        if name in self:
            return self[name]
        if name in ModelOutputs._LAZY and "_model" in self:
            m = self["_model"]
            if name == "pruned_prediction":
                self[name] = m.pruned_prediction(self)
            else:
                aux = m.aux_outputs(self)
                for k in aux:
                    self.setdefault(k, aux[k])
            if name in self:
                return self[name]
        raise AttributeError(name)


class PlanOpsMixin:

    def _buf(self, name, shape, dtype=torch.float32, zero=False):
        key = (self._buf_prefix + name, tuple(shape), dtype)
        t = self._bufs.get(key)
        if t is None:
            t = (torch.zeros if zero else torch.empty)(tuple(shape), dtype=dtype, device=self.device)
            self._bufs[key] = t
        return t

    @staticmethod
    def _rowsrc(ptr, sb, sr, width, shift=0, rowidx=None, scale=None, shiftv=None, act=0, cmod=0):
        s = rt.RowSrc()
        s.ptr, s.rowidx = ptr, (rowidx.data_ptr() if rowidx is not None else None)
        s.scale = scale.data_ptr() if scale is not None else None
        s.shiftv = shiftv.data_ptr() if shiftv is not None else None
        s.sb, s.sr, s.width, s.shift, s.act, s.cmod = sb, sr, width, shift, act, cmod
        return s

    @staticmethod
    def _dense_rows(srcs, rpb, M):
        if rpb != 1 or M == 1 or any(s.shift != 0 for s in srcs):
            return srcs, rpb, False
        out = []
        for s in srcs:
            t = rt.RowSrc()
            t.ptr, t.rowidx, t.scale, t.shiftv = s.ptr, s.rowidx, s.scale, s.shiftv
            t.sb, t.sr = 0, (s.sr if s.rowidx else s.sb)
            t.width, t.shift, t.act, t.cmod = s.width, s.shift, s.act, s.cmod
            out.append(t)
        return out, M, True

    def _gemm_group(self, plan, name, group):
        if len(group) > 1:
            n = len(group)
            tab = (rt.GemmArgs * n)(*[a for _, a in group])
            dims = (C.c_int32 * (4 * n))()
            total = C.c_int32()
            if self.lib.gcpx_gemm_group_dims(tab, n, dims, C.byref(total)) == 0:
                raw = torch.frombuffer(bytearray(bytes(tab)), dtype=torch.uint8).to(self.device)
                dd = torch.tensor(list(dims), dtype=torch.int32, device=self.device)
                plan.keep += [raw, dd, tab]
                plan.add(name, self.lib.gcpx_gemm_group, raw.data_ptr(), dd.data_ptr(), n, total.value)
                return
        for nm, a in group:
            if a.epi == rt.EPI_GAUSS_SAMPLE:
                m, e = a.src[0], a.src[1]
                plan.add(nm, self.lib.gcpx_gauss_sample, m.ptr, m.sb, m.sr, e.ptr, e.sb, e.sr, a.out, a.ob, a.orow, a.M, a.rpb, a.N)
            else:
                plan.add(nm, self.lib.gcpx_gemm, C.byref(a))

    def _gemm(self, plan, name, srcs, M, N, rpb, wpk, bias, out=None, ob=0, orow=0, epi=rt.EPI_NONE,
              stats=None, lstm=None, batch=None, group=None, lstm_bwd=None):
        srcs, rpb, dense = self._dense_rows(srcs, rpb, M)
        if dense:
            ob, orow = 0, ob
            if lstm is not None:
                c_prev, c_prev_stride, h_out, c_out, hb, hrow, h_copy = lstm
                lstm = (c_prev, c_prev_stride, h_out, c_out, 0, hb, h_copy)
        a = rt.GemmArgs()
        for i, s in enumerate(srcs):
            a.src[i] = s
        a.nsrc, a.M, a.N, a.K, a.rpb = len(srcs), M, N, sum(s.width for s in srcs), rpb
        a.wpk, a.bias = wpk.data_ptr(), (bias.data_ptr() if bias is not None else None)
        gs = self._gsplit.get(wpk.data_ptr())
        if gs is not None and self.split_f16 and (self._arena is None or self._gsplit_live):
            a.wpk_split, a.w_split_log2_dev = gs[0].data_ptr(), gs[1].data_ptr()
        a.out, a.ob, a.orow, a.epi = out, ob, orow, epi
        a.stats_partial = stats.data_ptr() if stats is not None else None
        if lstm is not None:
            a.c_prev, a.c_prev_stride, a.h_out, a.c_out, a.hb, a.hrow, a.h_copy = lstm
            if self.save_for_backward:
                g = self._buf(f"gates.{name}", (M, N))
                a.gates_out = g.data_ptr()
                plan.rec[f"gates:{name}"] = g
        if batch is not None:
            a.nbatch, a.z_src_off, a.z_w_off, a.z_bias_off, a.z_out_off = batch
        if lstm_bwd is not None:
            a.lstm_bwd = lstm_bwd
        if a.wpk_split and M >= self._planes_min_rows and N >= 1024 and group is None and not a.stats_partial:
            nbytes, nexp = C.c_int64(), C.c_int64()
            rt.check(self.lib.gcpx_gemm_planes_workspace(M, a.K, a.nbatch, C.byref(nbytes), C.byref(nexp)), "planes workspace")
            wsb = self._buf(f"xplanes.l{plan.lane}", (nbytes.value,), torch.uint8)
            wse = self._buf(f"xexp.l{plan.lane}", (nexp.value,), torch.int32)
            a.x_planes, a.x_exp, a.x_planes_bytes = wsb.data_ptr(), wse.data_ptr(), nbytes.value
        plan.keep.append(a)
        if group is not None:
            group.append((name, a))
            return
        plan.add(name, self.lib.gcpx_gemm, C.byref(a))

    def _mlp(self, plan, name, W, srcs, M, rpb, out=None, ob=0, orow=0, oblk=0, out_split=0, gauss=None, group=None, tanh=False):
        hp = self._hp
        rec_srcs, rec_rpb = srcs, rpb
        srcs, rpb, dense = self._dense_rows(srcs, rpb, M)
        if dense:
            ob, orow = 0, ob
            if gauss is not None:
                eps, eb, erow, z, zb, zrow = gauss
                gauss = (eps, 0, eb, z, 0, zb)
        a = rt.MlpArgs()
        for i, s in enumerate(srcs):
            a.src[i] = s
        a.nsrc, a.M, a.rpb = len(srcs), M, rpb
        a.in_dim, a.mid, a.n_mid, a.out_dim = W["in_dim"], W["mid"], W["n_mid"], W["out_dim"]
        assert a.in_dim == sum(s.width for s in srcs), (name, a.in_dim)
        a.w_in, a.b_in = W["w_in"].data_ptr(), W["b_in"].data_ptr()
        if W["n_mid"]:
            a.w_mid, a.b_mid = W["w_mid"].data_ptr(), W["b_mid"].data_ptr()
            a.gn_gamma, a.gn_beta = W["gn_g"].data_ptr(), W["gn_b"].data_ptr()
        a.w_out, a.b_out = W["w_out"].data_ptr(), W["b_out"].data_ptr()
        a.gn_eps, a.lrelu_slope = hp.gn_eps, hp.leaky_slope
        a.out, a.ob, a.orow, a.oblk, a.out_split = out, ob, orow, oblk, out_split
        a.epi = rt.MLP_TANH if tanh else rt.MLP_PLAIN
        if gauss is not None:
            a.epi = rt.MLP_GAUSS
            a.eps, a.eb, a.erow, a.z, a.zb, a.zrow = gauss
        if self.save_for_backward:
            sv = self._buf(f"save.{name}", (1 + 2 * W["n_mid"], M, W["mid"]))
            a.save = sv.data_ptr()
            plan.rec[f"mlp:{name}"] = dict(W=W, srcs=rec_srcs, M=M, rpb=rec_rpb, save=sv)
        plan.keep.append(a)
        if group is not None:
            group.append((name, a))
            return
        plan.add(name, self.lib.gcpx_mlp, C.byref(a))

    def _mlp_group(self, plan, name, group, gemm=None):
        if len(group) == 1:
            if gemm is not None:
                plan.add(gemm[0], self.lib.gcpx_gemm, C.byref(gemm[1]))
            plan.add(group[0][0], self.lib.gcpx_mlp, C.byref(group[0][1]))
            return
        n = len(group)
        tab = (rt.MlpArgs * n)(*[a for _, a in group])
        dims = (C.c_int32 * (4 * n))()
        total = C.c_int32()
        rt.check(self.lib.gcpx_mlp_group_dims(tab, n, dims, C.byref(total)), name)
        raw = torch.frombuffer(bytearray(bytes(tab)), dtype=torch.uint8).to(self.device)
        dd = torch.tensor(list(dims), dtype=torch.int32, device=self.device)
        plan.keep += [raw, dd, tab]
        mid = group[0][1].mid
        if gemm is not None:
            if os.environ.get("GCPX_NO_LEVEL_PRE") is None and self.lib.gcpx_mlp_group_gemm_supported(C.byref(gemm[1]), total.value, mid):
                plan.add(f"{name}+{gemm[0]}", self.lib.gcpx_mlp_group_gemm, raw.data_ptr(), dd.data_ptr(), n, total.value, mid, C.byref(gemm[1]))
                return
            plan.add(gemm[0], self.lib.gcpx_gemm, C.byref(gemm[1]))
        plan.add(name, self.lib.gcpx_mlp_group, raw.data_ptr(), dd.data_ptr(), n, total.value, mid)

    def _bn(self, plan, tag, prefix, C_, stats, n_partial, pitch, count):
        sd, hp = self.sd, self._hp
        scale, shift = self._buf(f"{tag}.scale", (C_,)), self._buf(f"{tag}.shift", (C_,))
        g, b = sd[f"{prefix}.weight"], sd[f"{prefix}.bias"]
        if self.training:
            mean = rstd = None
            if self.save_for_backward:
                mean, rstd = self._buf(f"{tag}.mean", (C_,)), self._buf(f"{tag}.rstd", (C_,))
                plan.rec[f"bn:{tag}"] = dict(prefix=prefix, C=C_, count=count, scale=scale, shift=shift, mean=mean, rstd=rstd)
            plan.add(f"bn_finalize:{tag}", self.lib.gcpx_bn_finalize, stats.data_ptr(), n_partial, pitch, C_,
                     C.c_double(float(count)), g.data_ptr(), b.data_ptr(), C.c_float(hp.bn_eps), scale.data_ptr(),
                     shift.data_ptr(), None, None, C.c_float(0.0), rt.ptr(mean), rt.ptr(rstd))
        else:
            plan.add(f"bn_fold:{tag}", self.lib.gcpx_bn_fold, sd[f"{prefix}.running_mean"].data_ptr(),
                     sd[f"{prefix}.running_var"].data_ptr(), g.data_ptr(), b.data_ptr(), C.c_float(hp.bn_eps), C_,
                     scale.data_ptr(), shift.data_ptr())
        return scale, shift

    def _conv_args(self, srcs, F, Hin, Win, Hout, Wout, Cout, out_pitch, wpk, bias, out, upsample=0, out_act=0,
                   head_mode=rt.HEAD_RAW, images=None, stats=None):
        a = rt.ConvArgs()
        cin = 0
        for i, (t_ptr, C_, fdiv, scale, shift, act) in enumerate(srcs):
            s = a.src[i]
            s.ptr, s.C, s.frame_div, s.act = t_ptr, C_, fdiv, act
            s.scale = scale.data_ptr() if scale is not None else None
            s.shift = shift.data_ptr() if shift is not None else None
            cin += C_
        a.nsrc, a.F, a.Hin, a.Win, a.Hout, a.Wout, a.Cin, a.Cout = len(srcs), F, Hin, Win, Hout, Wout, cin, Cout
        a.out_pitch, a.upsample, a.out_act, a.head_mode = out_pitch, upsample, out_act, head_mode
        a.wpk, a.bias = wpk.data_ptr(), bias.data_ptr()
        a.out = out.data_ptr() if out is not None else None
        a.images = images.data_ptr() if images is not None else None
        a.stats_partial = stats.data_ptr() if stats is not None else None
        return a
```

### video-gcp_amd/runtime.py

```python
import ctypes as C
import os

_HERE = os.path.dirname(os.path.abspath(__file__))
LIB_PATH = os.path.join(_HERE, "libgcpx.so")

ACT_NONE, ACT_LRELU, ACT_TANH = 0, 1, 2
HEAD_RAW, HEAD_DLM_MEAN, HEAD_DLM_BOTH, HEAD_TANH_NCHW, HEAD_DLM_NLL, HEAD_DLM_NLL_GRAD = 0, 1, 2, 3, 4, 5
SPLIT_PLAIN, SPLIT_ROWFOLD, SPLIT_HEAD32 = 0, 1, 2
EPI_NONE, EPI_LRELU, EPI_LSTM, EPI_GAUSS_SAMPLE = 0, 1, 2, 3
MLP_PLAIN, MLP_GAUSS, MLP_TANH = 0, 1, 2

vp = C.c_void_p
i32 = C.c_int32
i64 = C.c_int64


class ConvSrc(C.Structure):
    _fields_ = [("ptr", vp), ("scale", vp), ("shift", vp), ("C", i32), ("frame_div", i32), ("act", i32), ("_pad", i32)]


class ConvArgs(C.Structure):
    _fields_ = [("src", ConvSrc * 2), ("nsrc", i32), ("F", i32), ("Hin", i32), ("Win", i32), ("Hout", i32),
                ("Wout", i32), ("Cin", i32), ("Cout", i32), ("out_pitch", i32), ("upsample", i32), ("out_act", i32),
                ("head_mode", i32), ("wpk", vp), ("bias", vp), ("out", vp), ("images", vp), ("stats_partial", vp),
                ("raw_row_map", vp), ("src_row_map", vp), ("src_row_frames", vp), ("n_src_rows", i32), ("w_split_log2", i32), ("wpk_split", vp), ("w_split_log2_dev", vp),
                ("split_layout", i32), ("nll_rows", i32), ("nll_target", vp), ("nll_partial", vp), ("nll_row_weight", vp),
                ("nll_scale", C.c_float), ("_pad3", i32), ("images_rows", vp), ("images_rows_dup", i64), ("bwd_r", vp), ("bwd_scale", vp), ("bwd_shift", vp), ("bwd_mean", vp),
                ("bwd_rstd", vp), ("addend", vp), ("addend_frame_div", i32), ("_pad4", i32)]


class LossArgs(C.Structure):
    _fields_ = [("nll_bt", vp), ("pad_mask", vp), ("kl_b", vp), ("len_logits", vp), ("end_ind", vp), ("existence", vp),
                ("leave", vp), ("regressed_state", vp), ("state_target", vp), ("seq_len", vp), ("out", vp),
                ("B", i32), ("T", i32), ("N", i32), ("state_dim", i32), ("w_rec", C.c_float), ("w_kl", C.c_float),
                ("w_len", C.c_float), ("w_exist", C.c_float), ("w_state", C.c_float), ("total_div", C.c_float),
                ("action_pred", vp), ("action_seq", vp), ("inv_t0", vp), ("cost_pred", vp), ("cost_target", vp),
                ("n_actions", i32), ("w_action", C.c_float), ("w_cost", C.c_float), ("state_mask", vp), ("w_kl_dev", vp)]


class RowSrc(C.Structure):
    _fields_ = [("ptr", vp), ("rowidx", vp), ("scale", vp), ("shiftv", vp), ("sb", i64), ("sr", i64),
                ("width", i32), ("shift", i32), ("act", i32), ("cmod", i32)]


class GemmArgs(C.Structure):
    _fields_ = [("src", RowSrc * 6), ("nsrc", i32), ("M", i32), ("N", i32), ("K", i32), ("rpb", i32),
                ("wpk", vp), ("bias", vp), ("out", vp), ("ob", i64), ("orow", i64), ("epi", i32), ("nbatch", i32),
                ("stats_partial", vp), ("c_prev", vp), ("c_prev_stride", i64), ("h_out", vp), ("c_out", vp),
                ("hb", i64), ("hrow", i64), ("h_copy", vp), ("z_src_off", i64), ("z_w_off", i64),
                ("z_bias_off", i64), ("z_out_off", i64), ("gates_out", vp),
                ("wpk_split", vp), ("w_split_log2_dev", vp), ("w_split_log2", i32), ("_pad_split", i32),
                ("x_planes", vp), ("x_exp", vp), ("x_planes_bytes", i64), ("lstm_bwd", vp)]


class MlpArgs(C.Structure):
    _fields_ = [("src", RowSrc * 6), ("nsrc", i32), ("M", i32), ("rpb", i32), ("in_dim", i32), ("mid", i32),
                ("n_mid", i32), ("out_dim", i32), ("w_in", vp), ("b_in", vp), ("w_mid", vp), ("b_mid", vp),
                ("gn_gamma", vp), ("gn_beta", vp), ("w_out", vp), ("b_out", vp), ("gn_eps", C.c_float),
                ("lrelu_slope", C.c_float), ("epi", i32), ("out_split", i32), ("out", vp), ("ob", i64), ("orow", i64),
                ("oblk", i64), ("eps", vp), ("eb", i64), ("erow", i64), ("z", vp), ("zb", i64), ("zrow", i64), ("save", vp)]


class MlpBwdDx(C.Structure):
    _fields_ = [("wT", vp), ("out", vp), ("ob", i64), ("orow", i64), ("width", i32), ("_pad", i32)]


class MlpBwdArgs(C.Structure):
    _fields_ = [("dout", vp), ("save", vp), ("wT_out", vp), ("wT_mid", vp * 4), ("gn_gamma", vp * 4), ("gn_beta", vp * 4),
                ("du", vp * 5), ("gn_partial", vp * 4), ("dx", MlpBwdDx * 4), ("ldo", i64), ("M", i32), ("rpb", i32),
                ("mid", i32), ("n_mid", i32), ("out_pad", i32), ("ndx", i32), ("gn_eps", C.c_float), ("lrelu_slope", C.c_float)]


class SplitPackDesc(C.Structure):
    _fields_ = [("src", vp), ("idx", vp), ("out", vp), ("log2_out", vp), ("n", i32), ("_pad", i32)]


class WgradArgs(C.Structure):
    _fields_ = [("dy", vp), ("x", vp), ("rowidx", vp), ("frame_map", vp), ("scale", vp), ("shiftv", vp), ("out", vp),
                ("ldy", i64), ("sb", i64), ("sr", i64), ("ldw", i64), ("dy_sb", i64), ("R", i32), ("N", i32), ("n_valid", i32),
                ("K", i32), ("mode", i32), ("Cin", i32), ("H", i32), ("W", i32), ("rpb", i32), ("shift", i32),
                ("act", i32), ("cmod", i32), ("k_off", i32), ("accumulate", i32), ("partial", i32), ("nsplit", i32),
                ("dy_rpb", i32), ("nbatch", i32), ("dbias", vp), ("dbias2", vp), ("z_dy_off", i64), ("z_x_off", i64),
                ("z_out_off", i64), ("z_bias_off", i64), ("split_f16", i32), ("_pad_split", i32)]


class LstmBwdArgs(C.Structure):
    _fields_ = [("gates", vp), ("c_prev", vp), ("c_new", vp), ("dh_dense", vp), ("dh_pos", vp), ("dc_pos", vp),
                ("dgates", vp), ("dc_prev", vp), ("c_prev_stride", i64), ("pb", i64), ("prow", i64), ("dh_stride", i64),
                ("dcp_stride", i64), ("M", i32), ("H", i32), ("rpb", i32), ("_pad", i32)]


class TreeAccumSrc(C.Structure):
    _fields_ = [("ptr", vp), ("ld", i64), ("off_left", i32), ("off_right", i32), ("off_ctx0", i32), ("off_ctxg", i32),
                ("dst_col", i32), ("_pad", i32)]


class TreeAccumArgs(C.Structure):
    _fields_ = [("src", TreeAccumSrc * 6), ("dst", vp), ("dst_sb", i64), ("slot_stride", i64), ("nsrc", i32), ("B", i32),
                ("n", i32), ("width", i32)]


class ActBwdArgs(C.Structure):
    _fields_ = [("da", vp), ("add", vp), ("r", vp), ("scale", vp), ("shift", vp), ("mean", vp), ("rstd", vp), ("dy", vp),
                ("stats_partial", vp), ("ldc", i64), ("c_off", i32), ("up", i32), ("fsum", i32), ("act", i32), ("F", i32),
                ("H", i32), ("W", i32), ("C", i32)]


class PanelTile(C.Structure):
    _fields_ = [("kind", i32), ("src", i32), ("index", i32), ("length", i32), ("flags", i32), ("nb", i32), ("nf", i32),
                ("h", i32), ("w", i32), ("tile_w", i32), ("n0", i32), ("n_b", i32), ("n_f", i32), ("r0", i32), ("r_b", i32),
                ("r_f", i32), ("c0", i32), ("c_b", i32), ("c_f", i32), ("index_off", i32), ("index_stride", i32),
                ("index_count", i32), ("fill", C.c_float), ("_pad", i32), ("off", i64), ("s_b", i64), ("s_f", i64), ("s_c", i64),
                ("s_y", i64)]


PANEL_MAX_SRCS = 16
PANEL_IMAGE, PANEL_GREY, PANEL_GREY_ADD, PANEL_FILL = 0, 1, 2, 3
PANEL_RESCALE, PANEL_LENGTH_STRICT, PANEL_INDEX_FRAME, PANEL_INDEX_I64, PANEL_LENGTH_I64 = 1, 2, 4, 8, 16

WG_ROWS, WG_CONV1D, WG_CONV3X3, WG_CONV4X4S2 = 0, 1, 2, 3
WMAP_LINEAR, WMAP_CONV, WMAP_CONVT = 0, 1, 2

SYMBOLS = [
    ("gcpx_version", C.c_int, []),
    ("gcpx_last_error", C.c_char_p, []),
    ("gcpx_conv_grid", C.c_int, []),
    ("gcpx_conv3x3", C.c_int, [C.POINTER(ConvArgs), vp]),
    ("gcpx_conv3x3_grid", C.c_int, [C.POINTER(ConvArgs)]),
    ("gcpx_conv4x4s2", C.c_int, [C.POINTER(ConvArgs), vp]),
    ("gcpx_conv4x4s2_grid", C.c_int, []),
    ("gcpx_conv4x4s2_image", C.c_int, [vp, vp, vp, vp, i32, i32, i32, i32, i32, vp]),
    ("gcpx_bn_finalize", C.c_int, [vp, i32, i32, i32, C.c_double, vp, vp, C.c_float, vp, vp, vp, vp, C.c_float, vp, vp, vp]),
    ("gcpx_bn_fold", C.c_int, [vp, vp, vp, vp, C.c_float, i32, vp, vp, vp]),
    ("gcpx_randn", C.c_int, [vp, i64, vp, vp]),
    ("gcpx_gemm", C.c_int, [C.POINTER(GemmArgs), vp]),
    ("gcpx_gemm_row_blocks", C.c_int, [i32, i32]),
    ("gcpx_gemm_planes_workspace", C.c_int, [i32, i32, i32, vp, vp]),
    ("gcpx_mlp", C.c_int, [C.POINTER(MlpArgs), vp]),
    ("gcpx_balanced_binding", C.c_int, [vp, i32, i32, i32, vp, vp, vp, vp, vp, vp, vp]),
    ("gcpx_dlm_nll", C.c_int, [vp, vp, vp, vp, i32, i32, i32, i32, vp]),
    ("gcpx_gauss_nll", C.c_int, [vp, vp, vp, vp, i32, i32, vp]),
    ("gcpx_kl_gauss", C.c_int, [vp, vp, i32, i32, i32, i64, i64, C.c_float, vp, i64, vp, vp]),
    ("gcpx_gauss_sample", C.c_int, [vp, i64, i64, vp, i64, i64, vp, i64, i64, i32, i32, i32, vp]),
    ("gcpx_seq_index", C.c_int, [vp, i32, i32, vp, vp, vp]),
    ("gcpx_fill_zero", C.c_int, [vp, i64, vp]),
    ("gcpx_copy_rows", C.c_int, [vp, vp, i32, i32, i64, i64, i64, vp]),
    ("gcpx_loss_combine", C.c_int, [C.POINTER(LossArgs), vp]),
    ("gcpx_loss_pre", C.c_int, [C.POINTER(LossArgs), vp, vp, i32, i32, i64, i64, C.c_float, vp, i64, vp, vp]),
    ("gcpx_loss_final", C.c_int, [C.POINTER(LossArgs), vp]),
    ("gcpx_gather_rows", C.c_int, [vp, vp, vp, i32, i32, i32, i32, i64, vp]),
    ("gcpx_gather_rows_rest", C.c_int, [vp, vp, vp, i32, i32, i32, i32, i64, vp, vp]),
    ("gcpx_compact_index", C.c_int, [vp, i32, i32, i32, vp, vp]),
    ("gcpx_seq_pairs", C.c_int, [vp, vp, vp, vp, i32, i32, i32, vp]),
    ("gcpx_rollout_cost", C.c_int, [vp, i64, vp, vp, i64, vp, i32, i32, i32, i32, i32, C.c_float, vp]),
    ("gcpx_masked_row_sum", C.c_int, [vp, vp, vp, i32, i32, vp]),
    ("gcpx_wgrad", C.c_int, [C.POINTER(WgradArgs), vp]),
    ("gcpx_wgrad_classify", C.c_int, [C.POINTER(WgradArgs), i32, C.POINTER(C.c_int32), C.POINTER(C.c_int32)]),
    ("gcpx_wgrad_group", C.c_int, [vp, vp, i32, i32, i32, vp]),
    ("gcpx_wgrad_conv3x3", C.c_int, [vp, i32, vp, i32, i32, i32, i32, i32, vp, i32, vp]),
    ("gcpx_wgrad_conv3x3_split", C.c_int, [vp, i32, vp, i32, i32, i32, i32, i32, vp, i32, vp]),
    ("gcpx_wgrad_conv3x3_split_up", C.c_int, [vp, i32, C.POINTER(ConvArgs), i32, vp, i32, vp]),
    ("gcpx_wgrad_conv3x3_split_src", C.c_int, [vp, i32, vp, vp, vp, vp, i32, i32, i32, i32, i32, vp, vp, i32, vp]),
    ("gcpx_wgrad_image4x4s2", C.c_int, [vp, vp, vp, vp, i32, i32, vp, i32, vp]),
    ("gcpx_split_pack_group", C.c_int, [vp, i32, vp]),
    ("gcpx_split_pack_group2", C.c_int, [vp, i32, vp, vp]),
    ("gcpx_wgrad_reduce", C.c_int, [vp, i32, i32, i32, vp, i32, i32, i32, i32, vp, i64, i32, i32, vp]),
    ("gcpx_colsum", C.c_int, [vp, i64, i32, i32, i32, i64, i32, vp, vp, vp, i32, vp]),
    ("gcpx_reduce_partials", C.c_int, [vp, i32, i64, i32, vp, i32, vp]),
    ("gcpx_lstm_bwd", C.c_int, [C.POINTER(LstmBwdArgs), vp]),
    ("gcpx_mlp_bwd", C.c_int, [C.POINTER(MlpBwdArgs), vp]),
    ("gcpx_mlp_bwd_group", C.c_int, [C.POINTER(MlpBwdArgs), i32, vp]),
    ("gcpx_mlp_bwd_blocks", C.c_int, [i32]),
    ("gcpx_gn_lrelu_bwd", C.c_int, [vp, vp, vp, vp, vp, vp, i32, i32, i32, C.c_float, C.c_float, vp]),
    ("gcpx_gn_bwd_blocks", C.c_int, [i32]),
    ("gcpx_tanh_bwd_rows", C.c_int, [vp, vp, vp, i64, i64, i32, i32, i32, vp]),
    ("gcpx_lrelu_bwd", C.c_int, [vp, vp, vp, i64, C.c_float, vp]),
    ("gcpx_kl_bwd", C.c_int, [vp, vp, vp, vp, i32, i32, i32, i64, i64, C.c_float, C.c_float, vp]),
    ("gcpx_kl_bwd_weighted", C.c_int, [vp, vp, vp, vp, i32, i32, i32, i64, i64, C.c_float, C.c_float, vp, i64, vp]),
    ("gcpx_kl_bwd_scheduled", C.c_int, [vp, vp, vp, vp, i32, i32, i32, i64, i64, C.c_float, C.c_float, vp, i64, vp, vp]),
    ("gcpx_rows_strided", C.c_int, [vp, i64, i64, vp, i64, i64, i32, i32, i32, i32, vp]),
    ("gcpx_latent_bwd", C.c_int, [vp, vp, vp, i64, i64, vp, i64, i64, vp, i64, vp, i64, vp, vp, i32, i32, i32, vp]),
    ("gcpx_tree_accum", C.c_int, [C.POINTER(TreeAccumArgs), vp]),
    ("gcpx_timestep_scatter", C.c_int, [vp, i64, i64, vp, vp, i32, i32, i32, i32, vp]),
    ("gcpx_add_rows", C.c_int, [vp, i64, i64, vp, vp, i32, i32, i32, vp]),
    ("gcpx_zero_unmapped_rows", C.c_int, [vp, i64, vp, i32, vp]),
    ("gcpx_index_offset", C.c_int, [vp, vp, i32, i32, i32, vp]),
    ("gcpx_index_inverse", C.c_int, [vp, i32, vp, i32, vp]),
    ("gcpx_act_bwd", C.c_int, [C.POINTER(ActBwdArgs), vp]),
    ("gcpx_act_bwd_blocks", C.c_int, []),
    ("gcpx_act_skip_bwd", C.c_int, [C.POINTER(ActBwdArgs), vp, i32, i32, i32, vp]),
    ("gcpx_bn_bwd_finalize", C.c_int, [vp, i32, i32, C.c_double, vp, vp, vp, vp, vp, i32, vp]),
    ("gcpx_bn_bwd_apply", C.c_int, [vp, vp, vp, vp, vp, i64, i32, vp]),
    ("gcpx_conv_stage", C.c_int, [C.POINTER(ConvArgs), vp]),
    ("gcpx_col2im4x4s2", C.c_int, [vp, vp, i32, i32, i32, i32, vp]),
    ("gcpx_im2col_image", C.c_int, [vp, vp, i32, i32, i32, vp]),
    ("gcpx_dlm_nll_bwd", C.c_int, [vp, vp, vp, C.c_float, vp, vp, vp, i32, i32, i32, i32, vp]),
    ("gcpx_loss_heads_bwd", C.c_int, [C.POINTER(LossArgs), vp, vp, vp, vp]),
    ("gcpx_image_metrics", C.c_int, [vp, vp, vp, vp, vp, i32, i32, i32, i32, i32, vp, vp, vp]),
    ("gcpx_topn_accumulate", C.c_int, [vp, i32, i32, i32, i32, i32, vp, vp, vp, i32, vp, vp, vp, i32, vp, vp, i32, vp, i32, vp, i64,
                                        vp]),
    ("gcpx_gemm_group_dims", C.c_int, [vp, i32, vp, vp]),
    ("gcpx_gemm_group", C.c_int, [vp, vp, i32, i32, vp]),
    ("gcpx_mlp_group_dims", C.c_int, [vp, i32, vp, vp]),
    ("gcpx_mlp_group", C.c_int, [vp, vp, i32, i32, i32, vp]),
    ("gcpx_mlp_group_gemm_supported", C.c_int, [C.POINTER(GemmArgs), i32, i32]),
# ... 100 lines not shown
```

### video-gcp_amd/weights.py

```python
import ctypes as C
import os
from contextlib import contextmanager

import torch

from . import packing as pk
from . import runtime as rt
from .hparams import GCPHParams
from .params import init_params, encoder_layers, encoder_skip_layers, decoder_layers
from .plan_ops import _addr


class WeightsMixin:

    def _flatten_params(self, params):
        off, self._poff = 0, {}
        for k, v in params.items():
            self._poff[k] = (off, tuple(v.shape))
            off += (v.numel() + 3) // 4 * 4
        self.theta = torch.zeros(off, dtype=torch.float32, device=self.device)
        self.sd = {}
        for k, v in params.items():
            o, shp = self._poff[k]
            view = self.theta[o:o + v.numel()].view(shp)
            view.copy_(v)
            self.sd[k] = view

    def _pack_predictor(self, prefix, out_dim):
        sd = self._psd
        mid = sd[f"{prefix}.input.linear.weight"].shape[0]
        n_mid = 0
        while f"{prefix}.pyramid-{n_mid}.linear.weight" in sd:
            n_mid += 1
        out_pad = (out_dim + 15) // 16 * 16
        w_in = sd[f"{prefix}.input.linear.weight"]
        k_raw = w_in.shape[1]
        if k_raw % 16:
            w_in = torch.cat([w_in, torch.zeros((mid, -k_raw % 16), dtype=w_in.dtype, device=w_in.device)], 1)
        d = dict(mid=mid, n_mid=n_mid, out_dim=out_dim, in_dim=w_in.shape[1], in_dim_raw=k_raw)
        d["w_in"] = pk.pack_gemm(w_in)
        d["b_in"] = sd[f"{prefix}.input.linear.bias"].contiguous()
        if n_mid:
            d["w_mid"] = torch.stack([pk.pack_gemm(sd[f"{prefix}.pyramid-{i}.linear.weight"]) for i in range(n_mid)]).contiguous()
            d["b_mid"] = torch.stack([sd[f"{prefix}.pyramid-{i}.linear.bias"] for i in range(n_mid)]).contiguous()
            d["gn_g"] = torch.stack([sd[f"{prefix}.pyramid-{i}.norm.weight"] for i in range(n_mid)]).contiguous()
            d["gn_b"] = torch.stack([sd[f"{prefix}.pyramid-{i}.norm.bias"] for i in range(n_mid)]).contiguous()
        d["w_out"] = pk.pack_gemm(sd[f"{prefix}.head.linear.weight"])
        d["b_out"] = pk.pad_vec(sd[f"{prefix}.head.linear.bias"], out_pad)
        return d

    def _pack_all(self):
        if self._arena is not None:
            self.repack()
            return
        self.pk = self._pack_tree(self.sd)
        if self._hp.tree_lstm:
            self._pack_fused_embed()
        self._pack_split()
        self._pack_gemm_split()

    def _pack_split(self):
        self.pk_split = {}
        hp = self._hp
        todo = []
        if hp.decoder_distribution == "discrete_logistic_mixture":
            todo.append(("dec.head", "decoder.gen_head.conv.weight", pk.dlm_channel_perm(hp.n_mixtures)))
            if self.head32 and hp.n_mixtures == 10 and hp.head_channels == 100:
                todo.append(("dec.head32", "decoder.gen_head.conv.weight", ("head32", pk.dlm_channel_perm(hp.n_mixtures))))
        for name, c_prev, c_skip, skip_idx, cout in decoder_layers(hp):
            if cout == 16 and c_prev + c_skip == 32:
                todo.append((f"dec.{name}", f"decoder.net.{name}.conv.weight", "rowfold"))
            elif cout == 16:
                todo.append((f"dec.{name}", f"decoder.net.{name}.conv.weight", None))
            elif cout in (32, 64) and (c_prev + c_skip) % 32 == 0:
                todo.append((f"dec.{name}", f"decoder.net.{name}.conv.weight", "tiled32"))
        for name, cin, cout, norm in self._enc_layers[1:]:
            if cin == 16 or cin % 32 == 0:
                todo.append((f"enc.{name}", f"encoder.net.{name}.conv.weight", "enc4x4"))
        for name, key, perm in todo:
            off, shp = self._poff[key]
            d = {}
            if perm == "enc4x4":
                idx = pk.conv4x4_split_index(shp, off).to(self.device)
            elif perm == "rowfold":
                d["fold"] = torch.zeros(24 * shp[0] * shp[1], dtype=torch.float32, device=self.device)
                d["fold_src"] = (off, shp[0], shp[1])
                idx = pk.conv3x3_fold_index().to(self.device)
            elif perm == "tiled32":
                idx = pk.conv3x3_split32_index(shp, off).to(self.device)
            elif isinstance(perm, tuple) and perm[0] == "head32":
                idx = pk.head32_index(shp, off, perm[1]).to(self.device)
            else:
                idx = pk.conv3x3_split_index(shp, off, perm).to(self.device)
            d.update(idx=idx, out=torch.zeros(2 * idx.numel(), dtype=torch.int16, device=self.device),
                     log2=torch.zeros(1, dtype=torch.int32, device=self.device))
            self.pk_split[name] = d
        self.repack_split()

    def repack_split(self, stream=None):
        st = stream if stream is not None else torch.cuda.current_stream(self.device).cuda_stream
        if not self.pk_split:
            return
        tab = self._split_tab
        key = (self.theta.data_ptr(),) + tuple((d["out"].data_ptr(), d["idx"].data_ptr()) for d in self.pk_split.values())
        if tab is None or tab[2] != key:
            descs = []
            for name, d in self.pk_split.items():
                src = d["fold"] if "fold" in d else self.theta
                e = rt.SplitPackDesc()
                e.src, e.idx, e.out, e.log2_out, e.n = src.data_ptr(), d["idx"].data_ptr(), d["out"].data_ptr(), d["log2"].data_ptr(), d["idx"].numel()
                descs.append(e)
            arr = (rt.SplitPackDesc * len(descs))(*descs)
            dev = torch.frombuffer(bytearray(bytes(arr)), dtype=torch.uint8).to(self.device)
            tab = self._split_tab = (dev, len(descs), key, torch.zeros(len(descs), dtype=torch.int32, device=self.device))
        for name, d in self.pk_split.items():
            if "fold_src" in d:
                off, cout, cin = d["fold_src"]
                rt.check(self.lib.gcpx_fold_upsample_weights(self.theta.data_ptr() + 4 * off, cout, cin, d["fold"].data_ptr(), st), "fold_upsample_weights")
        rt.check(self.lib.gcpx_split_pack_group2(tab[0].data_ptr(), tab[1], tab[3].data_ptr(), st), "split_pack_group2")

    def _pack_gemm_split(self):
        self._gsplit = {}
        self._merge_side_rows = int(os.environ.get("GCPX_MERGE_SIDE_ROWS", "512")) or (1 << 60)
        pr = int(os.environ.get("GCPX_GEMM_PLANES_ROWS", "512"))
        self._planes_min_rows = pr if pr > 0 else 1 << 60
        if not self.split_f16:
            return
        for name, W in self.pk.items():
            if not (isinstance(W, dict) and name.startswith("tree")):
                continue
            for key, wpk in W.items():
                if not (key.endswith(".w") and (key.startswith("lstm") or key == "proj.w")):
                    continue
                stack = wpk if wpk.dim() == 5 else wpk[None]
                if (stack.shape[2] * 16) % 64 or (stack.shape[1] * 16) % 64:
                    continue
                packs = [pk.pack_gemm_split(pk.unpack_gemm(w, w.shape[1] * 16)) for w in stack]
                ws = torch.stack([p_[0] for p_ in packs]).contiguous().to(self.device)
                es = torch.tensor([p_[1] for p_ in packs], dtype=torch.int32, device=self.device)
                self._gsplit[wpk.data_ptr()] = (ws, es)

    def _set_split(self, a, name):
        d = self.pk_split.get(name)
        layout = None
        if name == "dec.head" and self.head32 and a.head_mode in (rt.HEAD_DLM_MEAN, rt.HEAD_DLM_NLL, rt.HEAD_DLM_NLL_GRAD) \
                and "dec.head32" in self.pk_split:
            d, layout = self.pk_split["dec.head32"], rt.SPLIT_HEAD32
        if self.split_f16 and d is not None:
            a.wpk_split, a.w_split_log2_dev = d["out"].data_ptr(), d["log2"].data_ptr()
            if layout is None:
                layout = rt.SPLIT_ROWFOLD if "fold" in d else rt.SPLIT_PLAIN
            a.split_layout = layout

    def _pack_fused_embed(self):
        hp = self._hp
        for l in range(hp.hierarchy_levels if hp.untied_layers else 1):
            p = f"tree_module.tree_modules.{l}.subgoal_pred"
            sd = self.sd
            We, be = sd[f"{p}.embed.weight"].double(), sd[f"{p}.embed.bias"].double()
            Wih = sd[f"{p}.lstm.0.weight_ih"].double()
            Wf = (Wih @ We).float()
            bf = (Wih @ be).float() + sd[f"{p}.lstm.0.bias_ih"]
            w, b = pk.lstm_gate_interleave(Wf, sd[f"{p}.lstm.0.weight_hh"], bf, sd[f"{p}.lstm.0.bias_hh"])
            self.pk[f"tree{l}"]["lstm0f.w"], self.pk[f"tree{l}"]["lstm0f.b"] = pk.pack_gemm(w), b

    def _pack_tree(self, sd):
        hp = self._hp
        self._psd = sd
        P = {}
        layers, c_top = encoder_layers(hp)
        self._enc_layers, self._c_top = layers, c_top
        P["enc.input.w"] = pk.pack_conv4x4_image(sd["encoder.net.input.conv.weight"])
        P["enc.input.b"] = sd["encoder.net.input.conv.bias"].contiguous()
        for name, cin, cout, norm in layers[1:]:
            P[f"enc.{name}.w"] = pk.pack_conv4x4(sd[f"encoder.net.{name}.conv.weight"])
            P[f"enc.{name}.b"] = sd[f"encoder.net.{name}.conv.bias"].contiguous()
        wh = sd["encoder.net.head.weight"]
        P["enc.head.w"] = pk.pack_gemm(wh.permute(0, 2, 3, 1).reshape(hp.nz_enc, 16 * c_top))
        P["enc.head.b"] = sd["encoder.net.head.bias"].contiguous()
        wt = sd["decoder.net.input.conv.weight"]
        P["dec.input.w"] = pk.pack_gemm(wt.permute(2, 3, 1, 0).reshape(16 * c_top, hp.nz_enc))
        P["dec.input.b"] = sd["decoder.net.input.conv.bias"].repeat(16).contiguous()
        for name, c_prev, c_skip, skip_idx, cout in decoder_layers(hp):
            P[f"dec.{name}.w"] = pk.pack_conv3x3(sd[f"decoder.net.{name}.conv.weight"], 16 if cout == 16 else 32)
            P[f"dec.{name}.b"] = pk.pad_vec(sd[f"decoder.net.{name}.conv.bias"], (cout + 15) // 16 * 16)
        hw, hb = sd["decoder.gen_head.conv.weight"], sd["decoder.gen_head.conv.bias"]
        if hp.decoder_distribution == "discrete_logistic_mixture":
            perm = pk.dlm_channel_perm(hp.n_mixtures)
            self._dlm_perm = torch.tensor(perm, device=self.device)
            P["dec.head.w"] = pk.pack_dlm_head(hw, perm)
            bk = torch.zeros(len(perm), device=hb.device, dtype=hb.dtype)
            permd = self._dlm_perm.to(hb.device)
            valid = permd >= 0
            bk[valid] = hb[permd[valid]]
            P["dec.head.b"] = bk
            self._head_pitch = len(perm)
        else:
            P["dec.head.w"] = pk.pack_conv3x3(hw, 16)
            P["dec.head.b"] = pk.pad_vec(hb, 16)
            self._head_pitch = 16
        seq_encs = [("seq", "inf_encoder")] + ([("kseq", "inf_key_encoder.0")] if hp.attentive_inference else [])
        if hp.seq_enc == "none":
            seq_encs = []
        for tag, pre in seq_encs:
            for nm in ["input"] + [f"pyramid-{i}" for i in range(hp.conv_inf_enc_layers)] + ["head"]:
                w = sd[f"{pre}.net.{nm}.conv.weight"]
                P[f"{tag}.{nm}.w"] = pk.pack_gemm(w.permute(0, 2, 1).reshape(w.shape[0], -1))
                P[f"{tag}.{nm}.b"] = sd[f"{pre}.net.{nm}.conv.bias"].contiguous()
        if hp.attentive_inference:
            P["kseq.key.w"] = pk.pack_gemm(sd["inf_key_encoder.1.linear.weight"])
            P["kseq.key.b"] = sd["inf_key_encoder.1.linear.bias"].contiguous()
        if hp.regress_length:
            P["length_pred"] = self._pack_predictor("length_pred.p", hp.max_seq_len)
        if hp.attach_state_regressor:
            P["state_regressor"] = self._pack_predictor("state_regressor", hp.state_dim)
        if hp.attach_inv_mdl:
            P["inv_mdl"] = self._pack_predictor("inv_mdl.action_pred", hp.n_actions)
        if hp.attach_cost_mdl:
            P["cost_mdl"] = self._pack_predictor("cost_mdl.cost_pred", 1)
        self._pack_latent_model(P)
        return P

    def build_arena(self, extra_pack=None):
        dev = self.device
        def probe(only_hh):
            sd = {}
            for k, (o, shp) in self._poff.items():
                n = 1
                for d in shp:
                    n *= d
                hh = k.endswith("bias_hh")
                if hh == only_hh:
                    sd[k] = (torch.arange(n, device=dev, dtype=torch.float64) + (o + 1)).view(shp)
                else:
                    sd[k] = torch.zeros(shp, device=dev, dtype=torch.float64)
            P = self._pack_tree(sd)
            X = extra_pack(sd) if extra_pack is not None else {}
            return P, X
        (P0, X0), (P1, X1) = probe(False), probe(True)
        leaves = []
        def walk(d0, d1, path):
            for k in d0:
                if isinstance(d0[k], dict):
                    walk(d0[k], d1[k], path + (k,))
                elif torch.is_tensor(d0[k]):
                    leaves.append((path + (k,), d0, d0[k], d1[k]))
        walk(P0, P1, ("P",))
        walk(X0, X1, ("X",))
        from .dist import gradient_bucket_ranges
        ranges = gradient_bucket_ranges(self._poff, self._hp.hierarchy_levels, self._hp.untied_layers)
        rest = len(ranges) - 1
        def bucket_of(t0, t1):
            ids = torch.cat([t0.reshape(-1), t1.reshape(-1)])
            ids = ids[ids > 0] - 1
            if ids.numel() == 0:
                return rest
            lo, hi = int(ids.min()), int(ids.max())
            for i, (_, a, b) in enumerate(ranges):
                if a <= lo and hi < b:
                    return i
            return rest
        leaves = [lf + (bucket_of(lf[2], lf[3]),) for lf in leaves]
        leaves.sort(key=lambda lf: (bool((lf[3] > 0).any()), lf[4]))
        leaves = [lf[:4] + (lf[4],) for lf in leaves]
        total = sum((lf[2].numel() + 3) // 4 * 4 for lf in leaves)
        self._arena = torch.zeros(total, dtype=torch.float32, device=dev)
        idx0 = torch.full((total,), -1, dtype=torch.int32, device=dev)
        idx1 = torch.full((total,), -1, dtype=torch.int32, device=dev)
        off = 0
        self._arena_split = None
        runs = {}
        for path, holder, t0, t1, bkt in leaves:
            n = t0.numel()
            two = bool((t1 > 0).any())
            if self._arena_split is None and two:
                self._arena_split = off
            idx0[off:off + n] = (t0.reshape(-1) - 1).to(torch.int32)
            idx1[off:off + n] = (t1.reshape(-1) - 1).to(torch.int32)
# ... 105 lines not shown
```

Before: 505,900.

## Chain LSTM layers through pre-split f16 planes, skipping per-layer conversion launches

In the tree LSTM stacks, the first layer's conversion launch now also converts the previous hidden states for the later layers into their own plane buffers. Each layer's LSTM epilogue writes its new hidden output straight into the next layer's input planes with a fixed exponent, and the consumer rescales its accumulator at the seam between fixed-scale and row-scaled K chunks. This removes the split_rows conversion kernel and the h_copy write for later layers. Separately, grouped MLP launches now halve their column blocks until the total fits within half the CU count. The cost is more complex accumulation logic and a fixed-scale f16 split for hidden values, which may slightly change precision.

Result: faster. 511,800 (median of 6 runs) (+1.2%).

```diff
diff --git a/include/gcpx.h b/include/gcpx.h
--- a/include/gcpx.h
+++ b/include/gcpx.h
@@ -146,7 +146,29 @@
     int32_t* x_exp;
     int64_t x_planes_bytes;
     const struct gcpx_lstm_bwd_args* lstm_bwd;
+    int32_t x_seam;
+    int32_t x_ready;
+    void* emit_planes;
+    int64_t emit_bytes;
+    int32_t emit_k0;
+    int32_t emit_nks;
+    const struct gcpx_planes_job* x_jobs;
+    int32_t n_x_jobs;
+    int32_t _pad_jobs;
 } gcpx_gemm_args;
+
+#define GCPX_PLANES_SEAM_EXP 14
+#define GCPX_MAX_PLANES_JOBS 3
+typedef struct gcpx_planes_job {
+    gcpx_row_src src;
+    void* planes;
+    int32_t* exp;
+    int64_t planes_bytes;
+    int32_t ks0, nks;
+    const int32_t* w_split_log2_dev;
+    int32_t w_split_log2;
+    int32_t _pad;
+} gcpx_planes_job;
 
 int gcpx_gemm(const gcpx_gemm_args* a, void* stream);
 int gcpx_gemm_planes_workspace(int32_t M, int32_t K, int32_t nbatch, int64_t* planes_bytes, int64_t* n_exp);
diff --git a/video-gcp_amd/csrc/gemm.hip b/video-gcp_amd/csrc/gemm.hip
--- a/video-gcp_amd/csrc/gemm.hip
+++ b/video-gcp_amd/csrc/gemm.hip
@@ -9,6 +9,7 @@
 int gcpx_launch_gemm_split(const gcpx_gemm_args* a, hipStream_t stream);
 bool gcpx_gemm_planes_applies(const gcpx_gemm_args* a);
 int gcpx_launch_gemm_planes(const gcpx_gemm_args* a, hipStream_t stream);
+int gcpx_gemm_planes_chain_check(const gcpx_gemm_args* a);
 
 namespace {
 
@@ -218,6 +219,10 @@
     hipStream_t stream = reinterpret_cast<hipStream_t>(stream_);
     const int st = gemm_check(a);
     if (st != GCPX_OK) return st;
+    if (a->x_seam || a->x_ready || a->emit_planes || a->n_x_jobs || a->x_jobs) {
+        const int sc = gcpx_gemm_planes_chain_check(a);
+        return sc != GCPX_OK ? sc : gcpx_launch_gemm_planes(a, stream);
+    }
     {
         int pr_ = 1, cr_ = 1;
         if (!ks_block_choice(a, &pr_, &cr_)) {
diff --git a/video-gcp_amd/csrc/gemm_planes.hip b/video-gcp_amd/csrc/gemm_planes.hip
--- a/video-gcp_amd/csrc/gemm_planes.hip
+++ b/video-gcp_amd/csrc/gemm_planes.hip
@@ -19,6 +19,17 @@
     return __builtin_amdgcn_mfma_f32_16x16x32_f16(a, b, c, 0, 0, 0);
 }
 
+typedef _Float16 h4 __attribute__((ext_vector_type(4)));
+__device__ __forceinline__ void split_seam(const float v, _Float16& p1, _Float16& p2) {
+    const float f = v * (float)(1 << GCPX_PLANES_SEAM_EXP);
+    p1 = (_Float16)f;
+    p2 = (_Float16)fmaf((float)p1, -1.f, f);
+}
+__device__ __forceinline__ char* emit_ptr(const gcpx_gemm_args& a, const int r, const int k) {
+    return reinterpret_cast<char*>(a.emit_planes) + ((size_t)(r >> 4) * a.emit_nks + (k >> 5)) * 2048 + ((((k & 31) >> 3) * 16 + (r & 15)) * 16) +
+           (k & 7) * 2;
+}
+
 __host__ __device__ __forceinline__ int padded_row_tiles(const int M) { return ((M + 255) >> 8) << 4; }
 
 __device__ __forceinline__ float sigmoid_hw(const float x) { return __builtin_amdgcn_rcpf(1.f + __builtin_amdgcn_exp2f(-1.44269504088896341f * x)); }
@@ -40,14 +51,29 @@
     for (int c = 0; c < 4; ++c) x[c] = __uint_as_float(u[c]);
 }
 
+struct split_prob {
+    gcpx_row_src src[6];
+    int nsrc, ks0, nks, ks_fixed;
+    char* planes;
+    int32_t* exp;
+    const int32_t* ew_dev;
+    long long ew;
+};
+struct split_tab {
+    split_prob p[1 + GCPX_MAX_PLANES_JOBS];
+    long long z_src_off;
+    int M, rpb;
+};
+
 template <bool XF, int NWV>
-__global__ void __launch_bounds__(64 * NWV) split_rows_kernel(const gcpx_gemm_args a) {
+__global__ void __launch_bounds__(64 * NWV) split_rows_kernel(const split_tab t) {
     __shared__ unsigned wmax[NWV][16];
     const int tid = threadIdx.x, lane = tid & 63, wave = tid >> 6;
     const int j = lane & 15, q = lane >> 4;
     const int zb = blockIdx.z, rt = blockIdx.x;
-    const int M = a.M, rpb = a.rpb;
-    const int NKS = a.K >> 5;
+    const split_prob& a = t.p[blockIdx.y];
+    const int M = t.M, rpb = t.rpb;
+    const int NKS = a.nks;
     const int r = rt * 16 + j;
     const bool rv = r < M;
     const int rs = rv ? r : 0;
@@ -68,7 +94,7 @@
                     ok = ok && jj >= 0 && jj < rpb;
                     off = (size_t)rb * src.sb + (size_t)(ok ? jj : 0) * src.sr;
                 }
-                const float* p = src.ptr + (size_t)zb * a.z_src_off + off + q * 8;
+                const float* p = src.ptr + (size_t)zb * t.z_src_off + off + q * 8;
                 const float mask = ok ? 1.f : 0.f;
                 const int n = src.width >> 5;
                 for (int l = (wave - s0) & (NWV - 1); l < n; l += NWV) {
@@ -82,7 +108,7 @@
                     }
                     v0.x *= mask; v0.y *= mask; v0.z *= mask; v0.w *= mask;
                     v1.x *= mask; v1.y *= mask; v1.z *= mask; v1.w *= mask;
-                    f(s0 + l, v0, v1);
+                    f(s0 + l, s0 + l < a.ks_fixed, v0, v1);
                 }
                 s0 += n;
             }
@@ -90,7 +116,8 @@
     };
 
     float amax = 0.f;
-    for_each_chunk([&](const int, const float4 v0, const float4 v1) {
+    for_each_chunk([&](const int, const bool fixed, const float4 v0, const float4 v1) {
+        if (fixed) return;
         amax = fmaxf(amax, fmaxf(fmaxf(fmaxf(fabsf(v0.x), fabsf(v0.y)), fmaxf(fabsf(v0.z), fabsf(v0.w))),
                                  fmaxf(fmaxf(fabsf(v1.x), fabsf(v1.y)), fmaxf(fabsf(v1.z), fabsf(v1.w)))));
     });
@@ -107,15 +134,16 @@
         for (int w = 1; w < NWV; ++w) u = max(u, wmax[w][j]);
         amax = __uint_as_float(u);
     }
-    const int ew = a.w_split_log2_dev ? a.w_split_log2_dev[zb] : a.w_split_log2;
+    const int ew = a.ew_dev ? a.ew_dev[zb] : (int)a.ew;
     const int ex_cap = min(100, 126 - ew);
     int ex = ex_cap;
     if (amax > 0.f) ex = min(ex_cap, max(-100, 14 + 127 - (int)((__float_as_uint(amax) >> 23) & 0xff)));
     if (!(amax < 3.0e38f)) ex = -100;
-    const float sc = __uint_as_float((unsigned)(127 + ex) << 23);
+    const float sc_row = __uint_as_float((unsigned)(127 + ex) << 23);
     const int RTP = padded_row_tiles(M);
-    char* dst = reinterpret_cast<char*>(a.x_planes) + (((size_t)zb * RTP + rt) * NKS) * 2048 + lane * 16;
-    for_each_chunk([&](const int ks, const float4 v0, const float4 v1) {
+    char* dst = a.planes + (((size_t)zb * RTP + rt) * NKS + a.ks0) * 2048 + lane * 16;
+    for_each_chunk([&](const int ks, const bool fixed, const float4 v0, const float4 v1) {
+        const float sc = fixed ? (float)(1 << GCPX_PLANES_SEAM_EXP) : sc_row;
         const float f[8] = {v0.x * sc, v0.y * sc, v0.z * sc, v0.w * sc, v1.x * sc, v1.y * sc, v1.z * sc, v1.w * sc};
         h8 p1, p2;
 #pragma unroll
@@ -126,7 +154,7 @@
         *reinterpret_cast<h8*>(dst + (size_t)ks * 2048) = p1;
         *reinterpret_cast<h8*>(dst + (size_t)ks * 2048 + 1024) = p2;
     });
-    if (wave == 0 && q == 0) a.x_exp[(size_t)zb * RTP * 16 + r] = ex;
+    if (wave == 0 && q == 0) a.exp[(size_t)zb * RTP * 16 + r] = ex;
 }
 
 __device__ __forceinline__ void glds16(const char* base, const unsigned voff, const unsigned lds_dst) {
@@ -139,7 +167,7 @@
     asm volatile("s_waitcnt vmcnt(%0)" ::"n"(N) : "memory");
 }
 
-template <int RT, int CTN, int NW, int WR, int KSUB, int STAGES, bool LSTM>
+template <int RT, int CTN, int NW, int WR, int KSUB, int STAGES, bool LSTM, bool SEAM>
 __global__ void __launch_bounds__(64 * NW) gemm_planes_kernel(const gcpx_gemm_args a, const int nbx, const int nby) {
     constexpr int WC = NW / WR, RPW = RT / WR, CPW = CTN / WC;
     constexpr int SUB_PIECES = (RT + CTN) * 2;
@@ -229,6 +257,7 @@
 #pragma unroll
     for (int s = 0; s < STAGES - 1; ++s)
         if (s < NK) issue(s, s);
+    const int s_seam = SEAM ? a.x_seam / (32 * KSUB) : -1;
     int buf = 0;
     for (int s = 0; s < NK; ++s) {
         if (s + STAGES - 2 < NK) wait_vm<(STAGES - 2) * LPS>();
@@ -242,6 +271,18 @@
         const long long tr0 = __builtin_amdgcn_s_memtime();
         __builtin_amdgcn_sched_barrier(0);
 #endif
+        if constexpr (SEAM) {
+            if (s == s_seam) {
+#pragma unroll
+                for (int i = 0; i < RPW; ++i) {
+                    const int r = (bx * RT + wr * RPW + i) * 16 + j;
+                    const int ex = a.x_exp[(size_t)zb * RTP * 16 + (r < M ? r : 0)];
+                    const float f = __uint_as_float((unsigned)(127 + ex - GCPX_PLANES_SEAM_EXP) << 23);
+#pragma unroll
+                    for (int c = 0; c < CPW; ++c) acc[c][i] *= f;
+                }
+            }
+        }
 #if GP_ABLATE != 2
         compute(buf);
 #endif
@@ -300,6 +341,18 @@
 #ifndef GP_TRACE
                     if (a.h_copy) *reinterpret_cast<float4*>(a.h_copy + (size_t)r * (a.N / 4) + u4) = make_float4(hv[0], hv[1], hv[2], hv[3]);
 #endif
+                    if (a.emit_planes) {
+                        h4 p1, p2;
+#pragma unroll
+                        for (int e = 0; e < 4; ++e) {
+                            _Float16 a1, a2;
+                            split_seam(hv[e], a1, a2);
+                            p1[e] = a1; p2[e] = a2;
+                        }
+                        char* d = emit_ptr(a, r, a.emit_k0 + u4);
+                        *reinterpret_cast<h4*>(d) = p1;
+                        *reinterpret_cast<h4*>(d + 1024) = p2;
+                    }
                 }
             }
             return;
@@ -335,6 +388,13 @@
 #ifndef GP_TRACE
                 if (a.h_copy) a.h_copy[(size_t)r * (a.N / 4) + u] = h;
 #endif
+                if (a.emit_planes) {
+                    _Float16 p1, p2;
+                    split_seam(h, p1, p2);
+                    char* d = emit_ptr(a, r, a.emit_k0 + u);
+                    *reinterpret_cast<_Float16*>(d) = p1;
+                    *reinterpret_cast<_Float16*>(d + 1024) = p2;
+                }
             } else {
                 if (a.epi == GCPX_EPI_LRELU) {
                     v[0] = lrelu(v[0], 0.2f); v[1] = lrelu(v[1], 0.2f); v[2] = lrelu(v[2], 0.2f); v[3] = lrelu(v[3], 0.2f);
@@ -351,8 +411,10 @@
     constexpr int LDS = STAGES * KSUB * (RT + CTN) * 2048;
     static bool attr_set = false;
     if (!attr_set) {
-        for (const void* k : {reinterpret_cast<const void*>(gemm_planes_kernel<RT, CTN, NW, WR, KSUB, STAGES, false>),
-                              reinterpret_cast<const void*>(gemm_planes_kernel<RT, CTN, NW, WR, KSUB, STAGES, true>)}) {
+        for (const void* k : {reinterpret_cast<const void*>(gemm_planes_kernel<RT, CTN, NW, WR, KSUB, STAGES, false, false>),
+                              reinterpret_cast<const void*>(gemm_planes_kernel<RT, CTN, NW, WR, KSUB, STAGES, true, false>),
+                              reinterpret_cast<const void*>(gemm_planes_kernel<RT, CTN, NW, WR, KSUB, STAGES, false, true>),
+                              reinterpret_cast<const void*>(gemm_planes_kernel<RT, CTN, NW, WR, KSUB, STAGES, true, true>)}) {
             hipError_t e = hipFuncSetAttribute(k, hipFuncAttributeMaxDynamicSharedMemorySize, LDS);
             if (e != hipSuccess) {
                 gcpx_set_error("gemm planes: hipFuncSetAttribute(%d B LDS): %s", LDS, hipGetErrorString(e));
@@ -364,10 +426,14 @@
     const int nb = a->nbatch > 1 ? a->nbatch : 1;
     const int nbx = (a->M + RT * 16 - 1) / (RT * 16), nby = a->N / (CTN * 16);
     const dim3 grid(nbx * nby, 1, nb);
-    if (a->epi == GCPX_EPI_LSTM)
-        hipLaunchKernelGGL((gemm_planes_kernel<RT, CTN, NW, WR, KSUB, STAGES, true>), grid, dim3(64 * NW), LDS, stream, *a, nbx, nby);
-    else
-        hipLaunchKernelGGL((gemm_planes_kernel<RT, CTN, NW, WR, KSUB, STAGES, false>), grid, dim3(64 * NW), LDS, stream, *a, nbx, nby);
+    const bool lstm = a->epi == GCPX_EPI_LSTM;
+    if (a->x_seam) {
+        if (lstm) hipLaunchKernelGGL((gemm_planes_kernel<RT, CTN, NW, WR, KSUB, STAGES, true, true>), grid, dim3(64 * NW), LDS, stream, *a, nbx, nby);
+        else hipLaunchKernelGGL((gemm_planes_kernel<RT, CTN, NW, WR, KSUB, STAGES, false, true>), grid, dim3(64 * NW), LDS, stream, *a, nbx, nby);
+    } else {
+        if (lstm) hipLaunchKernelGGL((gemm_planes_kernel<RT, CTN, NW, WR, KSUB, STAGES, true, false>), grid, dim3(64 * NW), LDS, stream, *a, nbx, nby);
+        else hipLaunchKernelGGL((gemm_planes_kernel<RT, CTN, NW, WR, KSUB, STAGES, false, false>), grid, dim3(64 * NW), LDS, stream, *a, nbx, nby);
+    }
     GCPX_CHECK_LAUNCH();
     return GCPX_OK;
 }
@@ -392,19 +458,74 @@
     return a->x_planes_bytes >= need;
 }
 
+int gcpx_gemm_planes_chain_check(const gcpx_gemm_args* a) {
+    GCPX_CHECK_ARG(gcpx_gemm_planes_applies(a), "seam / emission / conversion jobs need the planes form (workspace, split weights, >= 512 rows, N % 128 == 0, K % 64 == 0)");
+    GCPX_CHECK_ARG(a->nbatch <= 1, "seam / emission / conversion jobs: single problem only");
+    GCPX_CHECK_ARG(a->x_seam >= 0 && a->n_x_jobs >= 0 && a->n_x_jobs <= GCPX_MAX_PLANES_JOBS, "bad x_seam / n_x_jobs");
+    GCPX_CHECK_ARG(!a->x_ready || a->x_seam, "x_ready needs x_seam");
+    GCPX_CHECK_ARG(!a->n_x_jobs || (a->x_jobs && !a->x_ready), "conversion jobs need a table and a conversion launch to ride in");
+    if (a->x_seam) {
+        GCPX_CHECK_ARG(a->x_seam % 64 == 0 && a->x_seam < a->K && a->x_seam <= 2048, "x_seam: a multiple of 64, below K, at most 2048");
+        if (!a->x_ready) {
+            int k = 0;
+            bool at = false;
+            for (int s = 0; s < a->nsrc; ++s) { k += a->src[s].width; at = at || k == a->x_seam; }
+            GCPX_CHECK_ARG(at, "x_seam must be a source boundary");
+        }
+    }
+    if (a->emit_planes) {
+        GCPX_CHECK_ARG(a->epi == GCPX_EPI_LSTM, "emit_planes: LSTM epilogue only");
+        GCPX_CHECK_ARG(a->emit_nks > 0 && a->emit_nks % 2 == 0 && a->emit_k0 >= 0 && a->emit_k0 % 32 == 0 && a->emit_k0 + a->N / 4 <= 32 * a->emit_nks,
+                       "emit_k0 / emit_nks do not hold the hidden width");
+        int64_t need = 0;
+        gcpx_gemm_planes_workspace(a->M, 32 * a->emit_nks, 1, &need, nullptr);
+        GCPX_CHECK_ARG(a->emit_bytes >= need, "emit_planes allocation too small for the consumer's planes");
+        GCPX_CHECK_ARG((reinterpret_cast<uintptr_t>(a->emit_planes) & 15) == 0 && a->emit_planes != a->x_planes, "emit_planes: 16-byte aligned, not this problem's own planes");
+    }
+    for (int i = 0; i < a->n_x_jobs; ++i) {
+        const gcpx_planes_job& jb = a->x_jobs[i];
+        GCPX_CHECK_ARG(jb.src.ptr && jb.planes && jb.exp && !jb.src.scale && !jb.src.act, "conversion job: NULL pointer or affine / activation");
+        GCPX_CHECK_ARG(jb.src.width > 0 && jb.src.width % 32 == 0 && jb.nks > 0 && jb.nks % 2 == 0 && jb.ks0 >= 0 && jb.ks0 + jb.src.width / 32 <= jb.nks,
+                       "conversion job: width / ks0 / nks");
+        int64_t need = 0;
+        gcpx_gemm_planes_workspace(a->M, 32 * jb.nks, 1, &need, nullptr);
+        GCPX_CHECK_ARG(jb.planes_bytes >= need && (reinterpret_cast<uintptr_t>(jb.planes) & 15) == 0, "conversion job: planes allocation too small or unaligned");
+    }
+    return GCPX_OK;
+}
+
 int gcpx_launch_gemm_planes(const gcpx_gemm_args* a, hipStream_t stream) {
     const int nb = a->nbatch > 1 ? a->nbatch : 1;
-    bool xf = false;
-    for (int s = 0; s < a->nsrc; ++s) xf = xf || a->src[s].scale || a->src[s].act;
-    const dim3 sgrid((a->M + 15) / 16, 1, nb);
-    if ((long)sgrid.x * nb >= 1024) {
-        if (xf) hipLaunchKernelGGL((split_rows_kernel<true, 4>), sgrid, dim3(256), 0, stream, *a);
-        else hipLaunchKernelGGL((split_rows_kernel<false, 4>), sgrid, dim3(256), 0, stream, *a);
-    } else {
-        if (xf) hipLaunchKernelGGL((split_rows_kernel<true, 16>), sgrid, dim3(1024), 0, stream, *a);
-        else hipLaunchKernelGGL((split_rows_kernel<false, 16>), sgrid, dim3(1024), 0, stream, *a);
-    }
-    GCPX_CHECK_LAUNCH();
+    if (!a->x_ready) {
+        split_tab t = {};
+        bool xf = false;
+        split_prob& p0 = t.p[0];
+        for (int s = 0; s < a->nsrc; ++s) {
+            xf = xf || a->src[s].scale || a->src[s].act;
+            p0.src[s] = a->src[s];
+        }
+        p0.nsrc = a->nsrc; p0.ks0 = 0; p0.nks = a->K / 32; p0.ks_fixed = a->x_seam / 32;
+        p0.planes = reinterpret_cast<char*>(a->x_planes); p0.exp = a->x_exp;
+        p0.ew_dev = a->w_split_log2_dev; p0.ew = a->w_split_log2;
+        for (int i = 0; i < a->n_x_jobs; ++i) {
+            const gcpx_planes_job& jb = a->x_jobs[i];
+            split_prob& p = t.p[1 + i];
+            p.src[0] = jb.src;
+            p.nsrc = 1; p.ks0 = jb.ks0; p.nks = jb.nks; p.ks_fixed = 0;
+            p.planes = reinterpret_cast<char*>(jb.planes); p.exp = jb.exp;
+            p.ew_dev = jb.w_split_log2_dev; p.ew = jb.w_split_log2;
+        }
+        t.z_src_off = a->z_src_off; t.M = a->M; t.rpb = a->rpb;
+        const dim3 sgrid((a->M + 15) / 16, 1 + a->n_x_jobs, nb);
+        if ((long)sgrid.x * sgrid.y * nb >= 1024) {
+            if (xf) hipLaunchKernelGGL((split_rows_kernel<true, 4>), sgrid, dim3(256), 0, stream, t);
+            else hipLaunchKernelGGL((split_rows_kernel<false, 4>), sgrid, dim3(256), 0, stream, t);
+        } else {
+            if (xf) hipLaunchKernelGGL((split_rows_kernel<true, 16>), sgrid, dim3(1024), 0, stream, t);
+            else hipLaunchKernelGGL((split_rows_kernel<false, 16>), sgrid, dim3(1024), 0, stream, t);
+        }
+        GCPX_CHECK_LAUNCH();
+    }
     static const int force = [] { const char* e = getenv("GCPX_GEMM_PLANES_CFG"); return e ? atoi(e) : 0; }();
     const long tiles_a = (long)((a->M + 255) / 256) * (a->N / 256) * nb, tiles_b = (long)((a->M + 127) / 128) * (a->N / 256) * nb;
     const long tiles_d = (long)((a->M + 127) / 128) * (a->N / 128) * nb;
diff --git a/video-gcp_amd/csrc/mlp.hip b/video-gcp_amd/csrc/mlp.hip
--- a/video-gcp_amd/csrc/mlp.hip
+++ b/video-gcp_amd/csrc/mlp.hip
@@ -383,8 +383,22 @@
         GCPX_CHECK_ARG(host_table[p].mid == host_table[0].mid, "all problems of a group share the hidden width");
         int gx, gy;
         mlp_grid(host_table + p, &gx, &gy);
-        dims[4 * p] = start; dims[4 * p + 1] = gx; dims[4 * p + 2] = gy; dims[4 * p + 3] = 0;
-        start += gx * gy;
+        dims[4 * p + 1] = gx; dims[4 * p + 2] = gy; dims[4 * p + 3] = 0;
+    }
+    const int cus = gcpx_conv_grid() / 2;
+    for (;;) {
+        int total = 0, widest = 1;
+        for (int p = 0; p < n; ++p) {
+            total += dims[4 * p + 1] * dims[4 * p + 2];
+            if (dims[4 * p + 2] > widest) widest = dims[4 * p + 2];
+        }
+        if (total <= cus || widest == 1) break;
+        for (int p = 0; p < n; ++p)
+            if (dims[4 * p + 2] == widest) dims[4 * p + 2] = widest / 2;
+    }
+    for (int p = 0; p < n; ++p) {
+        dims[4 * p] = start;
+        start += dims[4 * p + 1] * dims[4 * p + 2];
     }
     *total_blocks = start;
     return GCPX_OK;
diff --git a/video-gcp_amd/forward_plan.py b/video-gcp_amd/forward_plan.py
--- a/video-gcp_amd/forward_plan.py
+++ b/video-gcp_amd/forward_plan.py
@@ -345,17 +345,20 @@
             fused = "lstm0f.w" in W and not self.save_for_backward
             if not fused:
                 self._gemm(plan, f"embed{l}", srcs, M, H, n, W["embed.w"], W["embed.b"], out=x.data_ptr(), ob=n * H, orow=H)
+            h_prev = lambda i: self._rowsrc(_addr(merged, 2 * i * H), n * 2 * nl * H, 2 * nl * H, H)
+            chain = {"nl": nl, "later": [(h_prev(i), W[f"lstm{i}.w"]) for i in range(1, nl)]}
             for i in range(nl):
                 xn = self._buf(f"x{l}.{i + 1}", (M, H))
                 xs = self._rowsrc(x.data_ptr(), n * H, H, H)
-                hs = self._rowsrc(_addr(merged, 2 * i * H), n * 2 * nl * H, 2 * nl * H, H)
+                hs = h_prev(i)
+                chain["i"] = i
                 lstm = (_addr(merged, (2 * i + 1) * H), 2 * nl * H, _addr(Hid, nodeoff(SD) + 2 * i * H),
                         _addr(Hid, nodeoff(SD) + (2 * i + 1) * H), PS * SD, 2 * s * SD, xn.data_ptr())
                 if i == 0 and fused:
-                    self._gemm(plan, f"lstm{l}.0", srcs + [hs], M, 4 * H, n, W["lstm0f.w"], W["lstm0f.b"], epi=rt.EPI_LSTM, lstm=lstm)
+                    self._gemm(plan, f"lstm{l}.0", srcs + [hs], M, 4 * H, n, W["lstm0f.w"], W["lstm0f.b"], epi=rt.EPI_LSTM, lstm=lstm, chain=chain)
                 else:
                     self._gemm(plan, f"lstm{l}.{i}", [xs, hs], M, 4 * H, n, W[f"lstm{i}.w"], W[f"lstm{i}.b"],
-                               epi=rt.EPI_LSTM, lstm=lstm)
+                               epi=rt.EPI_LSTM, lstm=lstm, chain=chain)
                 x = xn
             g = []
             self._gemm(plan, f"out{l}", [self._rowsrc(x.data_ptr(), n * H, H, H)], M, nz, n, W["out.w"], W["out.b"],
diff --git a/video-gcp_amd/model.py b/video-gcp_amd/model.py
--- a/video-gcp_amd/model.py
+++ b/video-gcp_amd/model.py
@@ -42,6 +42,7 @@
         self._gsplit_live = False
         self._merge_side_rows = 1 << 60
         self._planes_min_rows = 1 << 60
+        self._lstm_planes_chain = True
         self._arena = None
         self._plan_listeners = []
         self._rng_seed = None
diff --git a/video-gcp_amd/plan_ops.py b/video-gcp_amd/plan_ops.py
--- a/video-gcp_amd/plan_ops.py
+++ b/video-gcp_amd/plan_ops.py
@@ -196,7 +196,7 @@
                 plan.add(nm, self.lib.gcpx_gemm, C.byref(a))
 
     def _gemm(self, plan, name, srcs, M, N, rpb, wpk, bias, out=None, ob=0, orow=0, epi=rt.EPI_NONE,
-              stats=None, lstm=None, batch=None, group=None, lstm_bwd=None):
+              stats=None, lstm=None, batch=None, group=None, lstm_bwd=None, chain=None):
         srcs, rpb, dense = self._dense_rows(srcs, rpb, M)
         if dense:
             ob, orow = 0, ob
@@ -229,11 +229,44 @@
             wsb = self._buf(f"xplanes.l{plan.lane}", (nbytes.value,), torch.uint8)
             wse = self._buf(f"xexp.l{plan.lane}", (nexp.value,), torch.int32)
             a.x_planes, a.x_exp, a.x_planes_bytes = wsb.data_ptr(), wse.data_ptr(), nbytes.value
+            if chain is not None and self._lstm_planes_chain and epi == rt.EPI_LSTM and not dense and a.nbatch <= 1:
+                self._chain_planes(plan, a, chain)
         plan.keep.append(a)
         if group is not None:
             group.append((name, a))
             return
         plan.add(name, self.lib.gcpx_gemm, C.byref(a))
+
+    def _chain_planes(self, plan, a, chain):
+        i, nl, H = chain["i"], chain["nl"], a.N // 4
+        if i == 0:
+            later = [(hs, self._gsplit.get(wpk.data_ptr())) for hs, wpk in chain["later"]]
+            if not (1 <= len(later) <= rt.MAX_PLANES_JOBS and H % 64 == 0 and H <= 2048 and all(gs is not None and hs.width == H for hs, gs in later)):
+                return
+            nbytes, nexp = C.c_int64(), C.c_int64()
+            rt.check(self.lib.gcpx_gemm_planes_workspace(a.M, 2 * H, 1, C.byref(nbytes), C.byref(nexp)), "planes workspace")
+            jobs, ws = (rt.PlanesJob * len(later))(), []
+            for t, (hs, gs) in enumerate(later, 1):
+                wsb = self._buf(f"xplanes.l{plan.lane}.layer{t}", (nbytes.value,), torch.uint8, zero=True)
+                wse = self._buf(f"xexp.l{plan.lane}.layer{t}", (nexp.value,), torch.int32, zero=True)
+                jb = jobs[t - 1]
+                jb.src, jb.planes, jb.exp, jb.planes_bytes = hs, wsb.data_ptr(), wse.data_ptr(), nbytes.value
+                jb.ks0, jb.nks, jb.w_split_log2_dev = H // 32, 2 * H // 32, gs[1].data_ptr()
+                ws.append((wsb, wse, nbytes.value))
+            a.x_jobs, a.n_x_jobs = C.addressof(jobs), len(later)
+            plan.keep.append(jobs)
+            chain["ws"] = ws
+        elif "ws" in chain:
+            wsb, wse, nb = chain["ws"][i - 1]
+            a.x_planes, a.x_exp, a.x_planes_bytes = wsb.data_ptr(), wse.data_ptr(), nb
+            a.x_seam, a.x_ready = H, 1
+        else:
+            return
+        if i + 1 < nl:
+            wsb, _, nb = chain["ws"][i]
+            a.emit_planes, a.emit_bytes, a.emit_k0, a.emit_nks = wsb.data_ptr(), nb, 0, 2 * H // 32
+            if not self.save_for_backward:
+                a.h_copy = None
 
     def _mlp(self, plan, name, W, srcs, M, rpb, out=None, ob=0, orow=0, oblk=0, out_split=0, gauss=None, group=None, tanh=False):
         hp = self._hp
diff --git a/video-gcp_amd/runtime.py b/video-gcp_amd/runtime.py
--- a/video-gcp_amd/runtime.py
+++ b/video-gcp_amd/runtime.py
@@ -50,7 +50,17 @@
                 ("hb", i64), ("hrow", i64), ("h_copy", vp), ("z_src_off", i64), ("z_w_off", i64),
                 ("z_bias_off", i64), ("z_out_off", i64), ("gates_out", vp),
                 ("wpk_split", vp), ("w_split_log2_dev", vp), ("w_split_log2", i32), ("_pad_split", i32),
-                ("x_planes", vp), ("x_exp", vp), ("x_planes_bytes", i64), ("lstm_bwd", vp)]
+                ("x_planes", vp), ("x_exp", vp), ("x_planes_bytes", i64), ("lstm_bwd", vp),
+                ("x_seam", i32), ("x_ready", i32), ("emit_planes", vp), ("emit_bytes", i64), ("emit_k0", i32), ("emit_nks", i32),
+                ("x_jobs", vp), ("n_x_jobs", i32), ("_pad_jobs", i32)]
+
+
+class PlanesJob(C.Structure):
+    _fields_ = [("src", RowSrc), ("planes", vp), ("exp", vp), ("planes_bytes", i64), ("ks0", i32), ("nks", i32),
+                ("w_split_log2_dev", vp), ("w_split_log2", i32), ("_pad", i32)]
+
+
+PLANES_SEAM_EXP, MAX_PLANES_JOBS = 14, 3
 
 
 class MlpArgs(C.Structure):
diff --git a/video-gcp_amd/weights.py b/video-gcp_amd/weights.py
--- a/video-gcp_amd/weights.py
+++ b/video-gcp_amd/weights.py
@@ -124,6 +124,7 @@
         self._merge_side_rows = int(os.environ.get("GCPX_MERGE_SIDE_ROWS", "512")) or (1 << 60)
         pr = int(os.environ.get("GCPX_GEMM_PLANES_ROWS", "512"))
         self._planes_min_rows = pr if pr > 0 else 1 << 60
+        self._lstm_planes_chain = os.environ.get("GCPX_LSTM_PLANES_CHAIN", "1") != "0"
         if not self.split_f16:
             return
         for name, W in self.pk.items():
```
